# cbacary/MoDeGPT

Measured on AMD Instinct MI355X. Metric: transformer layers compressed/sec (covariance+decomp+rebuild), Llama-3-8B @30%, higher is better.
Workload: dtype f64 from int8 MFMA digit planes, exact route: nine plane pairs + fp64 remainder sums, nothing truncated (error <= 5e-15 per call: fp64 rounding)

## Files before the change

### modegpt_amd/csrc/common.hpp

```cpp
#pragma once
#include <hip/hip_runtime.h>
#include <hip/hip_bf16.h>
#include <hip/hip_fp16.h>
#include <stdint.h>
#include <stdio.h>
#include <string.h>

#include "../../include/modegpt_hip.h"

namespace mdg {

typedef double d4 __attribute__((ext_vector_type(4)));
typedef double d2 __attribute__((ext_vector_type(2)));
typedef unsigned short bf16_t;
typedef unsigned short f16_t;

#ifdef MDG_EXPERIMENT
#define MDG_KNOB(name) (getenv(name) != nullptr)
#else
#define MDG_KNOB(name) false
#endif

void set_error(const char* fmt, ...);
enum { STATUS_NOT_PD = 1, STATUS_NO_CONVERGE = 2 };
int finish_flag(int* dflag, hipStream_t st, int kind, const char* what);

int release_i8_schedules();
int cov_accum_gated(const void* x, int dtype, int64_t n_tokens, int64_t n_feat, int64_t batch, int64_t ld, int relu, double* sigma,
                    int64_t ld_sigma, int64_t sigma_bs, void* ws, size_t ws_bytes, const int* gate, int gate_mask, int gate_want,
                    void* stream);
#define MDG_CHECK_ARG(cond, ...)            \
  do {                                      \
    if (!(cond)) {                          \
      mdg::set_error(__VA_ARGS__);          \
      return MDG_ERR_BAD_ARG;               \
    }                                       \
  } while (0)
#define MDG_HIP(call)                                                        \
  do {                                                                       \
    hipError_t e_ = (call);                                                  \
    if (e_ != hipSuccess) {                                                  \
      mdg::set_error("%s failed: %s (%s:%d)", #call, hipGetErrorString(e_),  \
                     __FILE__, __LINE__);                                    \
      return MDG_ERR_HIP;                                                    \
    }                                                                        \
  } while (0)
#define MDG_LAUNCH_CHECK() MDG_HIP(hipGetLastError())
#define MDG_CLEAR() (void)hipGetLastError()
#define MDG_TRY(call)              \
  do {                             \
    int s_ = (call);               \
    if (s_ != MDG_OK) return s_;   \
  } while (0)

__device__ __forceinline__ double bf16_to_f64(bf16_t b) {
  return (double)__uint_as_float(((unsigned)b) << 16);
}
__device__ __forceinline__ double f16_to_f64(f16_t h) {
  __half_raw r;
  r.x = h;
  return (double)__half2float(__half(r));
}
__device__ __forceinline__ bf16_t f64_to_bf16(double v) {
  float f = (float)v;
  unsigned u = __float_as_uint(f);
  if ((u & 0x7fffffffu) > 0x7f800000u) return (bf16_t)0x7fc0;
  u += 0x7fffu + ((u >> 16) & 1u);
  return (bf16_t)(u >> 16);
}

template <int DT> struct ElemOf;
template <> struct ElemOf<MDG_BF16> { typedef bf16_t type; };
template <> struct ElemOf<MDG_F16> { typedef f16_t type; };
template <> struct ElemOf<MDG_F32> { typedef float type; };
template <> struct ElemOf<MDG_F64> { typedef double type; };

template <int DT> __device__ __forceinline__ double load_f64(const void* p, int64_t i);
template <> __device__ __forceinline__ double load_f64<MDG_BF16>(const void* p, int64_t i) {
  return bf16_to_f64(((const bf16_t*)p)[i]);
}
template <> __device__ __forceinline__ double load_f64<MDG_F16>(const void* p, int64_t i) {
  return f16_to_f64(((const f16_t*)p)[i]);
}
template <> __device__ __forceinline__ double load_f64<MDG_F32>(const void* p, int64_t i) {
  return (double)((const float*)p)[i];
}
template <> __device__ __forceinline__ double load_f64<MDG_F64>(const void* p, int64_t i) {
  return ((const double*)p)[i];
}

static inline size_t dtype_size(int dt) {
  switch (dt) {
    case MDG_BF16: case MDG_F16: return 2;
    case MDG_F32: return 4;
    case MDG_F64: return 8;
  }
  return 0;
}

static inline int64_t ceil_div(int64_t a, int64_t b) { return (a + b - 1) / b; }
static inline size_t align_up(size_t a, size_t b) { return (a + b - 1) / b * b; }

constexpr int TILE = 128;
constexpr int WTILE = 64;
constexpr int BK = 16;
constexpr int PITCH = TILE + 2;
constexpr int PANEL = BK * PITCH;

struct Acc {
  d4 v[4][4];
};

__device__ __forceinline__ void acc_zero(Acc& a) {
#pragma unroll
  for (int i = 0; i < 4; i++)
#pragma unroll
    for (int j = 0; j < 4; j++) a.v[i][j] = (d4){0., 0., 0., 0.};
}

template <int K4_LO, int K4_HI>
__device__ __forceinline__ void mma_steps(const double* __restrict__ As, const double* __restrict__ Bs, int wr,
                                          int wc, int lane, Acc& acc) {
  const int m = lane & 15, kq = lane >> 4;
#pragma unroll
  for (int k4 = K4_LO; k4 < K4_HI; k4++) {
    const double* ap = As + (k4 * 4 + kq) * PITCH + wr * WTILE + 4 * m;
    const double* bp = Bs + (k4 * 4 + kq) * PITCH + wc * WTILE + 4 * m;
    d2 a01 = *(const d2*)ap, a23 = *(const d2*)(ap + 2);
    d2 b01 = *(const d2*)bp, b23 = *(const d2*)(bp + 2);
    double a[4] = {a01.x, a01.y, a23.x, a23.y};
    double b[4] = {b01.x, b01.y, b23.x, b23.y};
#pragma unroll
    for (int sa = 0; sa < 4; sa++)
#pragma unroll
      for (int sb = 0; sb < 4; sb++)
        acc.v[sa][sb] = __builtin_amdgcn_mfma_f64_16x16x4f64(a[sa], b[sb], acc.v[sa][sb], 0, 0, 0);
  }
}

__device__ __forceinline__ void mma_stage(const double* __restrict__ As, const double* __restrict__ Bs, int wr,
                                          int wc, int lane, Acc& acc) {
  mma_steps<0, BK / 4>(As, Bs, wr, wc, lane, acc);
}

__device__ __forceinline__ int acc_row(int wr, int lane, int sa, int reg) {
  return wr * WTILE + 4 * ((lane >> 4) + 4 * reg) + sa;
}
__device__ __forceinline__ int acc_col(int wc, int lane, int sb) { return wc * WTILE + 4 * (lane & 15) + sb; }

__device__ __forceinline__ void tri_decode(int t, int& bi, int& bj) {
  int i = (int)((sqrt(8.0 * (double)t + 1.0) - 1.0) * 0.5);
  while ((i + 1) * (i + 2) / 2 <= t) i++;
  while (i * (i + 1) / 2 > t) i--;
  bi = i;
  bj = t - i * (i + 1) / 2;
}

}
```

### modegpt_amd/csrc/cov.hip

```cpp
#include <stdlib.h>

#include <type_traits>

#include "common.hpp"

namespace mdg {

struct CovArgs {
  const void* x;
  int64_t ld, n_tokens;
  int n_feat, batch, tiles, ntri;
  double* sigma;
  int64_t ld_sigma, sigma_bs;
  int ksplit;
  int64_t tokens_per_split;
  double* partial;
  int vec_ok;
  const int* gate;
  int gate_mask, gate_want;
};

template <int DT> struct Stage {
  typedef typename ElemOf<DT>::type T;
  static constexpr int VEC = 16 / (int)sizeof(T);
  static constexpr int CPR = TILE / VEC;
  static constexpr int CPT = BK * CPR / 256;
  union Chunk {
    uint4 q;
    T e[VEC];
  };
  static constexpr int RG = VEC >= 8 ? 4 : (VEC == 4 ? 2 : 1);
  static constexpr int CG = 8 / RG;
  __device__ static __forceinline__ void chunk_rc(int c, int& row, int& col) {
    const int g = c >> 3, i = c & 7;
    row = (g % (BK / RG)) * RG + (i % RG);
    col = ((g / (BK / RG)) * CG + i / RG) * VEC;
  }
};

template <int DT, bool FAST, bool INB = false>
__device__ __forceinline__ void load_panel(const CovArgs& a, int64_t tok0, int64_t tok_end, int64_t col0,
                                           int col_lim, int tid, typename Stage<DT>::Chunk* regs) {
  typedef Stage<DT> S;
  typedef typename S::T T;
  const T* x = (const T*)a.x;
#pragma unroll
  for (int p = 0; p < S::CPT; p++) {
    int row, col;
    S::chunk_rc(tid + 256 * p, row, col);
    int64_t tok = tok0 + row;
    typename S::Chunk ch;
    ch.q = make_uint4(0, 0, 0, 0);
    if (FAST && INB) {
      ch.q = *(const uint4*)(x + tok * a.ld + col0 + col);
    } else if (FAST) {
      if (tok < tok_end) ch.q = *(const uint4*)(x + tok * a.ld + col0 + col);
    } else if (tok < tok_end) {
      const T* src = x + tok * a.ld + col0 + col;
      if (a.vec_ok && col + S::VEC <= col_lim) {
        ch.q = *(const uint4*)src;
      } else {
#pragma unroll
        for (int e = 0; e < S::VEC; e++)
          if (col + e < col_lim) ch.e[e] = src[e];
      }
    }
    regs[p] = ch;
  }
}

template <int DT, bool RELU>
__device__ __forceinline__ void store_panel(double* panel, int tid, const typename Stage<DT>::Chunk* regs) {
  typedef Stage<DT> S;
#pragma unroll
  for (int p = 0; p < S::CPT; p++) {
    int row, col;
    S::chunk_rc(tid + 256 * p, row, col);
    double* dst = panel + row * PITCH + col;
#pragma unroll
    for (int e = 0; e < S::VEC; e += 2) {
      double v0 = load_f64<DT>(regs[p].e, e), v1 = load_f64<DT>(regs[p].e, e + 1);
      if (RELU) {
        v0 = v0 > 0. ? v0 : 0.;
        v1 = v1 > 0. ? v1 : 0.;
      }
      *(d2*)(dst + e) = (d2){v0, v1};
    }
  }
}

template <int DT, bool RELU>
__device__ __forceinline__ void store_piece(double* panel, int tid, const typename Stage<DT>::Chunk* regs, int piece) {
  typedef Stage<DT> S;
  constexpr int PAIRS = S::CPT * S::VEC / 2;
  constexpr int PER = PAIRS / 4;
#pragma unroll
  for (int u = 0; u < PER; u++) {
    const int w = piece * PER + u;
    const int p = w / (S::VEC / 2), e = (w % (S::VEC / 2)) * 2;
    int row, col;
    S::chunk_rc(tid + 256 * p, row, col);
    double v0 = load_f64<DT>(regs[p].e, e), v1 = load_f64<DT>(regs[p].e, e + 1);
    if (RELU) {
      v0 = v0 > 0. ? v0 : 0.;
      v1 = v1 > 0. ? v1 : 0.;
    }
    *(d2*)(panel + row * PITCH + col + e) = (d2){v0, v1};
  }
}

template <int DT, bool RELU, bool DIAG>
__device__ __forceinline__ void mma_half_with_staging(const double* __restrict__ As, const double* __restrict__ Bs,
                                                      int wr, int wc, int lane, Acc& acc, bool stage_next,
                                                      double* nextA, double* nextB, int tid,
                                                      const typename Stage<DT>::Chunk* ra,
                                                      const typename Stage<DT>::Chunk* rb) {
  const int m = lane & 15, kq = lane >> 4;
  double a[2][4], b[2][4];
#pragma unroll
  for (int h = 0; h < 2; h++) {
    const int k4 = BK / 8 + h;
    const double* ap = As + (k4 * 4 + kq) * PITCH + wr * WTILE + 4 * m;
    const double* bp = Bs + (k4 * 4 + kq) * PITCH + wc * WTILE + 4 * m;
    d2 a01 = *(const d2*)ap, a23 = *(const d2*)(ap + 2);
    d2 b01 = *(const d2*)bp, b23 = *(const d2*)(bp + 2);
    a[h][0] = a01.x; a[h][1] = a01.y; a[h][2] = a23.x; a[h][3] = a23.y;
    b[h][0] = b01.x; b[h][1] = b01.y; b[h][2] = b23.x; b[h][3] = b23.y;
  }
#pragma unroll
  for (int h = 0; h < 2; h++)
#pragma unroll
    for (int sa = 0; sa < 4; sa++) {
#pragma unroll
      for (int sb = 0; sb < 4; sb++)
        acc.v[sa][sb] = __builtin_amdgcn_mfma_f64_16x16x4f64(a[h][sa], b[h][sb], acc.v[sa][sb], 0, 0, 0);
      if (stage_next) {
        const int piece = h * 4 + sa;
        if (piece < 4) store_piece<DT, RELU>(nextA, tid, ra, piece);
        else if (!DIAG) store_piece<DT, RELU>(nextB, tid, rb, piece - 4);
      }
      __builtin_amdgcn_sched_barrier(0);
    }
}

template <int DT, bool RELU, bool FAST, bool DIAG>
__device__ __forceinline__ void cov_tile(const CovArgs& a, double* lds, int b, int bi, int bj, int split, int slot) {
  typedef Stage<DT> S;
  const int tid = threadIdx.x, lane = tid & 63, wave = tid >> 6;
  const int wr = wave >> 1, wc = wave & 1;
  const int64_t tok_begin = (int64_t)split * a.tokens_per_split;
  int64_t tok_end = tok_begin + a.tokens_per_split;
  if (tok_end > a.n_tokens) tok_end = a.n_tokens;
  const int64_t colA = (int64_t)b * a.n_feat + (int64_t)bi * TILE;
  const int64_t colB = (int64_t)b * a.n_feat + (int64_t)bj * TILE;
  const int limA = min(TILE, a.n_feat - bi * TILE), limB = min(TILE, a.n_feat - bj * TILE);

  Acc acc;
  acc_zero(acc);
  typename S::Chunk ra1[S::CPT], rb1[S::CPT], ra2[S::CPT], rb2[S::CPT];
  const int64_t n_stage = tok_end > tok_begin ? (tok_end - tok_begin + BK - 1) / BK : 0;

  if (n_stage > 0) {
    load_panel<DT, FAST>(a, tok_begin, tok_end, colA, limA, tid, ra1);
    if (!DIAG) load_panel<DT, FAST>(a, tok_begin, tok_end, colB, limB, tid, rb1);
    store_panel<DT, RELU>(lds, tid, ra1);
    if (!DIAG) store_panel<DT, RELU>(lds + 2 * PANEL, tid, rb1);
    if (n_stage > 1) {
      load_panel<DT, FAST>(a, tok_begin + BK, tok_end, colA, limA, tid, ra1);
      if (!DIAG) load_panel<DT, FAST>(a, tok_begin + BK, tok_end, colB, limB, tid, rb1);
    }
  }
  __syncthreads();
  auto stage = [&](int64_t s, auto cur_c, auto steady_c, typename S::Chunk* st_a, typename S::Chunk* st_b,
                   typename S::Chunk* ld_a, typename S::Chunk* ld_b) {
    constexpr int CUR = decltype(cur_c)::value;
    constexpr bool STEADY = decltype(steady_c)::value;
    if (STEADY || s + 2 < n_stage) {
      const int64_t tk = tok_begin + (s + 2) * BK;
      load_panel<DT, FAST, STEADY>(a, tk, tok_end, colA, limA, tid, ld_a);
      if (!DIAG) load_panel<DT, FAST, STEADY>(a, tk, tok_end, colB, limB, tid, ld_b);
    }
    const double* As = lds + CUR * PANEL;
    const double* Bs = DIAG ? As : lds + (2 + CUR) * PANEL;
    mma_steps<0, BK / 8>(As, Bs, wr, wc, lane, acc);
    mma_half_with_staging<DT, RELU, DIAG>(As, Bs, wr, wc, lane, acc, STEADY || s + 1 < n_stage, lds + (CUR ^ 1) * PANEL,
                                          lds + (2 + (CUR ^ 1)) * PANEL, tid, st_a, st_b);
    __syncthreads();
  };
  using I0 = std::integral_constant<int, 0>;
  using I1 = std::integral_constant<int, 1>;
  int64_t s = 0;
  const int64_t n_full = (tok_end - tok_begin) / BK;
  for (; s + 3 < n_full; s += 2) {
    stage(s, I0{}, std::true_type{}, ra1, rb1, ra2, rb2);
    stage(s + 1, I1{}, std::true_type{}, ra2, rb2, ra1, rb1);
  }
  for (; s + 1 < n_stage; s += 2) {
    stage(s, I0{}, std::false_type{}, ra1, rb1, ra2, rb2);
    stage(s + 1, I1{}, std::false_type{}, ra2, rb2, ra1, rb1);
  }
  if (s < n_stage) stage(s, I0{}, std::false_type{}, ra1, rb1, ra2, rb2);

  if (a.ksplit == 1) {
    double* sg = a.sigma + (int64_t)b * a.sigma_bs;
#pragma unroll
    for (int sa = 0; sa < 4; sa++)
#pragma unroll
      for (int reg = 0; reg < 4; reg++) {
        int r = acc_row(wr, lane, sa, reg);
        int64_t gr = (int64_t)bi * TILE + r;
        if (gr >= a.n_feat) continue;
        int c0 = acc_col(wc, lane, 0);
        int64_t gc0 = (int64_t)bj * TILE + c0;
        double* row = sg + gr * a.ld_sigma + gc0;
#pragma unroll
        for (int sb = 0; sb < 4; sb++)
          if (gc0 + sb < a.n_feat) row[sb] += acc.v[sa][sb][reg];
      }
  } else {
    double* pt = a.partial + ((int64_t)split * (a.batch * a.ntri) + slot) * (TILE * TILE);
#pragma unroll
    for (int sa = 0; sa < 4; sa++)
#pragma unroll
      for (int reg = 0; reg < 4; reg++) {
        int r = acc_row(wr, lane, sa, reg);
        int c0 = acc_col(wc, lane, 0);
        d4 v = {acc.v[sa][0][reg], acc.v[sa][1][reg], acc.v[sa][2][reg], acc.v[sa][3][reg]};
        *(d4*)(pt + r * TILE + c0) = v;
      }
  }
}

template <int DT, bool RELU, bool FAST>
__global__ __launch_bounds__(256, 2) void cov_accum_kernel(CovArgs a) {
  __shared__ double lds[4 * PANEL];
  if (a.gate && (*a.gate & a.gate_mask) != a.gate_want) return;
  const int b = blockIdx.x / a.ntri, t = blockIdx.x % a.ntri;
  int bi, bj;
  tri_decode(t, bi, bj);
  if (bi == bj) cov_tile<DT, RELU, FAST, true>(a, lds, b, bi, bj, blockIdx.y, blockIdx.x);
  else cov_tile<DT, RELU, FAST, false>(a, lds, b, bi, bj, blockIdx.y, blockIdx.x);
}

constexpr int MULTI_MAX = 4;
struct CovMulti {
  int n;
  int unit_start[MULTI_MAX + 1];
  CovArgs p[MULTI_MAX];
};

template <int DT>
__global__ __launch_bounds__(256, 2) void cov_accum_multi_kernel(CovMulti m) {
  __shared__ double lds[4 * PANEL];
  int u = blockIdx.x, pi = 0;
  while (pi + 1 < m.n && u >= m.unit_start[pi + 1]) pi++;
  u -= m.unit_start[pi];
  const CovArgs& a = m.p[pi];
  const int tiles = a.batch * a.ntri;
  const int split = u / tiles, slot = u % tiles;
  const int b = slot / a.ntri, t = slot % a.ntri;
  int bi, bj;
  tri_decode(t, bi, bj);
  if (bi == bj) cov_tile<DT, false, true, true>(a, lds, b, bi, bj, split, slot);
  else cov_tile<DT, false, true, false>(a, lds, b, bi, bj, split, slot);
}

__global__ __launch_bounds__(256) void cov_reduce_kernel(CovArgs a) {
  if (a.gate && (*a.gate & a.gate_mask) != a.gate_want) return;
  const int b = blockIdx.x / a.ntri, t = blockIdx.x % a.ntri;
  int bi, bj;
  tri_decode(t, bi, bj);
  double* sg = a.sigma + (int64_t)b * a.sigma_bs;
  const int64_t tile_stride = (int64_t)gridDim.x * (TILE * TILE);
  const double* pt = a.partial + (int64_t)blockIdx.x * (TILE * TILE);
  const int e = blockIdx.y * 256 + threadIdx.x;
  const int r = e / TILE, c = e % TILE;
  const int64_t gr = (int64_t)bi * TILE + r, gc = (int64_t)bj * TILE + c;
  if (gr >= a.n_feat || gc >= a.n_feat) return;
  double s = 0.;
  for (int k = 0; k < a.ksplit; k++) s += pt[k * tile_stride + e];
  sg[gr * a.ld_sigma + gc] += s;
}

__global__ __launch_bounds__(256) void cov_finalize_kernel(double* sigma, int n, int64_t ld, int64_t bs, int tiles,
                                                           int ntri, double scale) {
  __shared__ double tl[32][33];
  const int b = blockIdx.x / ntri, t = blockIdx.x % ntri;
  int ti, tj;
  tri_decode(t, ti, tj);
  double* sg = sigma + (int64_t)b * bs;
  const int tx = threadIdx.x & 31, ty = threadIdx.x >> 5;
  for (int r = ty; r < 32; r += 8) {
    int gr = ti * 32 + r, gc = tj * 32 + tx;
    tl[r][tx] = (gr < n && gc < n) ? sg[(int64_t)gr * ld + gc] * scale : 0.;
  }
  __syncthreads();
  for (int r = ty; r < 32; r += 8) {
    int gr = ti * 32 + r, gc = tj * 32 + tx;
    if (gr < n && gc < n) {
      double v = (ti == tj && tx > r) ? tl[tx][r] : tl[r][tx];
      sg[(int64_t)gr * ld + gc] = v;
    }
    if (ti != tj) {
      int ur = tj * 32 + r, uc = ti * 32 + tx;
      if (ur < n && uc < n) sg[(int64_t)ur * ld + uc] = tl[tx][r];
    }
  }
}

template <int DT>
__global__ __launch_bounds__(256) void bi_partial_kernel(const void* xin, const void* xout, int64_t n_tokens,
                                                         int64_t d, int64_t ld, double* partial) {
  __shared__ double red[4];
  const int lane = threadIdx.x & 63, wave = threadIdx.x >> 6;
  double local = 0.;
  for (int64_t tok = (int64_t)blockIdx.x * 4 + wave; tok < n_tokens; tok += (int64_t)gridDim.x * 4) {
    double dot = 0., na = 0., nb = 0.;
    for (int64_t j = lane; j < d; j += 64) {
      double u = load_f64<DT>(xin, tok * ld + j), v = load_f64<DT>(xout, tok * ld + j);
      dot += u * v;
      na += u * u;
      nb += v * v;
    }
    for (int o = 32; o > 0; o >>= 1) {
      dot += __shfl_xor(dot, o);
      na += __shfl_xor(na, o);
      nb += __shfl_xor(nb, o);
    }
    const double eps = 1e-8;
    double den = fmax(sqrt(na), eps) * fmax(sqrt(nb), eps);
    local += 1.0 - dot / den;
  }
  if (lane == 0) red[wave] = local;
  __syncthreads();
  if (threadIdx.x == 0) partial[blockIdx.x] = red[0] + red[1] + red[2] + red[3];
}

__global__ void bi_final_kernel(const double* partial, int n, double* out) {
  if (threadIdx.x == 0 && blockIdx.x == 0) {
    double s = 0.;
    for (int i = 0; i < n; i++) s += partial[i];
    *out += s;
  }
}

static int cov_ksplit(int64_t n_tokens, int64_t n_feat, int64_t batch, int64_t* tokens_per_split) {
  const int64_t T = ceil_div(n_feat, TILE);
  const int64_t blocks = batch * T * (T + 1) / 2;
  const double slots = 512.0;
  const double us_per_token = 2.0 * TILE * TILE / (78.6e12 / slots) * 1e6;
  const double us_per_tile_rt = 2.0 * TILE * TILE * 8 / 4.0e12 * 1e6;
  int64_t max_split = n_tokens / (8 * BK);
  if (max_split < 1) max_split = 1;
  if (max_split > 256) max_split = 256;
  int64_t best = 1;
  double best_cost = 0.;
#ifdef MDG_EXPERIMENT
  if (const char* ev = getenv("MDG_COV_KSPLIT")) {
    const int64_t f = atoll(ev);
    if (f >= 1 && f <= max_split) {
      const int64_t tps = (int64_t)align_up((size_t)ceil_div(n_tokens, f), BK);
      *tokens_per_split = tps;
      return (int)ceil_div(n_tokens, tps);
    }
  }
#endif
  for (int64_t ks = 1; ks <= max_split; ks++) {
    const int64_t tps = (int64_t)align_up((size_t)ceil_div(n_tokens, ks), BK);
    const int64_t real = ceil_div(n_tokens, tps);
    if (real != ks) continue;
    double rounds = (double)ceil_div(blocks * ks, (int64_t)slots);
    double cost = rounds * (double)tps * us_per_token + (ks > 1 ? (double)(blocks * ks) * us_per_tile_rt + 3.0 : 0.);
    if (ks == 1 || cost < best_cost * (best == 1 ? 0.95 : 0.98)) {
      best = ks;
      best_cost = cost;
    }
  }
  int64_t tps = (int64_t)align_up((size_t)ceil_div(n_tokens > 0 ? n_tokens : 1, best), BK);
  *tokens_per_split = tps;
  return (int)ceil_div(n_tokens > 0 ? n_tokens : 1, tps);
}

template <int DT>
static void launch_cov(const CovArgs& a, int relu, bool fast, hipStream_t st) {
  dim3 grid(a.batch * a.ntri, a.ksplit);
  if (fast) {
    if (relu) hipLaunchKernelGGL((cov_accum_kernel<DT, true, true>), grid, dim3(256), 0, st, a);
    else hipLaunchKernelGGL((cov_accum_kernel<DT, false, true>), grid, dim3(256), 0, st, a);
  } else {
    if (relu) hipLaunchKernelGGL((cov_accum_kernel<DT, true, false>), grid, dim3(256), 0, st, a);
    else hipLaunchKernelGGL((cov_accum_kernel<DT, false, false>), grid, dim3(256), 0, st, a);
  }
}

}

using namespace mdg;

extern "C" size_t mdg_cov_accum_ws_bytes(int64_t n_tokens, int64_t n_feat, int64_t batch) {
  if (n_tokens <= 0 || n_feat <= 0 || batch <= 0) return 0;
  int64_t tps;
  int ks = cov_ksplit(n_tokens, n_feat, batch, &tps);
  if (ks == 1) return 0;
  int64_t T = ceil_div(n_feat, TILE);
  return (size_t)ks * batch * (T * (T + 1) / 2) * TILE * TILE * sizeof(double);
}

extern "C" int mdg_cov_accum(const void* x, int dtype, int64_t n_tokens, int64_t n_feat, int64_t batch,
                             int64_t ld, int relu, double* sigma, int64_t ld_sigma, int64_t sigma_bs, void* ws,
                             size_t ws_bytes, void* stream) {
  return mdg::cov_accum_gated(x, dtype, n_tokens, n_feat, batch, ld, relu, sigma, ld_sigma, sigma_bs, ws, ws_bytes, nullptr, 0, 0,
                              stream);
}

int mdg::cov_accum_gated(const void* x, int dtype, int64_t n_tokens, int64_t n_feat, int64_t batch, int64_t ld, int relu,
                         double* sigma, int64_t ld_sigma, int64_t sigma_bs, void* ws, size_t ws_bytes, const int* gate,
                         int gate_mask, int gate_want, void* stream) {
  MDG_CLEAR();
  MDG_CHECK_ARG(n_tokens >= 0 && n_feat > 0 && batch > 0, "mdg_cov_accum: bad sizes (tokens=%lld feat=%lld batch=%lld)",
                (long long)n_tokens, (long long)n_feat, (long long)batch);
  MDG_CHECK_ARG(dtype >= MDG_BF16 && dtype <= MDG_F64, "mdg_cov_accum: unknown dtype %d", dtype);
  MDG_CHECK_ARG(ld >= n_feat * batch, "mdg_cov_accum: ld %lld < batch*n_feat %lld", (long long)ld,
                (long long)(n_feat * batch));
  MDG_CHECK_ARG(ld_sigma >= n_feat, "mdg_cov_accum: ld_sigma %lld < n_feat", (long long)ld_sigma);
  MDG_CHECK_ARG(batch == 1 || sigma_bs >= n_feat * ld_sigma - (ld_sigma - n_feat),
                "mdg_cov_accum: sigma batch stride too small");
  MDG_CHECK_ARG(n_feat < (1 << 30) && batch * n_feat < (1ll << 31), "mdg_cov_accum: n_feat too large");
  if (n_tokens == 0) return MDG_OK;
  MDG_CHECK_ARG(x && sigma, "mdg_cov_accum: null pointer");
  hipStream_t st = (hipStream_t)stream;
  CovArgs a;
  a.x = x;
  a.ld = ld;
  a.n_tokens = n_tokens;
  a.n_feat = (int)n_feat;
  a.batch = (int)batch;
  a.tiles = (int)ceil_div(n_feat, TILE);
  a.ntri = a.tiles * (a.tiles + 1) / 2;
  a.sigma = sigma;
  a.ld_sigma = ld_sigma;
  a.sigma_bs = sigma_bs;
  a.ksplit = cov_ksplit(n_tokens, n_feat, batch, &a.tokens_per_split);
  a.partial = (double*)ws;
  a.gate = gate;
  a.gate_mask = gate_mask;
  a.gate_want = gate_want;
  size_t esz = dtype_size(dtype);
  a.vec_ok = ((uintptr_t)x % 16 == 0) && ((ld * esz) % 16 == 0) && ((n_feat * esz) % 16 == 0 || batch == 1);
  if (a.ksplit > 1) {
    size_t need = mdg_cov_accum_ws_bytes(n_tokens, n_feat, batch);
    MDG_CHECK_ARG(ws && ws_bytes >= need, "mdg_cov_accum: workspace %zu < required %zu", ws_bytes, need);
  }
  MDG_CHECK_ARG((int64_t)a.batch * a.ntri < (1ll << 31) && a.ksplit < 65536, "mdg_cov_accum: grid too large");
  const bool fast = a.vec_ok && (n_feat % TILE == 0);
  switch (dtype) {
    case MDG_BF16: launch_cov<MDG_BF16>(a, relu, fast, st); break;
    case MDG_F16: launch_cov<MDG_F16>(a, relu, fast, st); break;
    case MDG_F32: launch_cov<MDG_F32>(a, relu, fast, st); break;
    default: launch_cov<MDG_F64>(a, relu, fast, st); break;
  }
  MDG_LAUNCH_CHECK();
  if (a.ksplit > 1) {
    hipLaunchKernelGGL(cov_reduce_kernel, dim3(a.batch * a.ntri, TILE * TILE / 256), dim3(256), 0, st, a);
    MDG_LAUNCH_CHECK();
  }
  return MDG_OK;
}

static int multi_ksplit(int64_t n_tokens, int64_t* tokens_per_split) {
  int64_t ks = n_tokens / 4096;
  if (ks < 1) ks = 1;
  if (ks > 64) ks = 64;
  int64_t tps = (int64_t)align_up((size_t)ceil_div(n_tokens, ks), BK);
  *tokens_per_split = tps;
  return (int)ceil_div(n_tokens, tps);
}

static int multi_plan(int n, const mdg_cov_problem* pr, int dtype, CovMulti* m, size_t* ws_need) {
  MDG_CHECK_ARG(n >= 1 && n <= MULTI_MAX && pr, "mdg_cov_accum_multi: 1..%d problems", MULTI_MAX);
  MDG_CHECK_ARG(dtype >= MDG_BF16 && dtype <= MDG_F64, "mdg_cov_accum_multi: unknown dtype %d", dtype);
  const size_t esz = dtype_size(dtype);
  size_t off = 0;
  int64_t units = 0;
  m->n = n;
  for (int i = 0; i < n; i++) {
    const mdg_cov_problem& q = pr[i];
    MDG_CHECK_ARG(q.n_tokens > 0 && q.n_feat > 0 && q.batch > 0 && q.x && q.sigma, "mdg_cov_accum_multi: problem %d empty", i);
    MDG_CHECK_ARG(q.n_feat % TILE == 0 && q.ld >= q.n_feat * q.batch && q.ld_sigma >= q.n_feat,
                  "mdg_cov_accum_multi: problem %d needs n_feat %% 128 == 0 (got %lld) and consistent strides", i,
                  (long long)q.n_feat);
    MDG_CHECK_ARG((uintptr_t)q.x % 16 == 0 && (q.ld * esz) % 16 == 0,
                  "mdg_cov_accum_multi: problem %d is not 16-byte aligned (use mdg_cov_accum)", i);
    CovArgs& a = m->p[i];
    a.x = q.x; a.ld = q.ld; a.n_tokens = q.n_tokens; a.n_feat = (int)q.n_feat; a.batch = (int)q.batch;
    a.tiles = (int)(q.n_feat / TILE); a.ntri = a.tiles * (a.tiles + 1) / 2;
    a.sigma = q.sigma; a.ld_sigma = q.ld_sigma; a.sigma_bs = q.sigma_batch_stride; a.vec_ok = 1;
    a.gate = nullptr; a.gate_mask = a.gate_want = 0;
    const int64_t tiles = (int64_t)a.batch * a.ntri;
    if (i == 0 && tiles >= 768) { a.ksplit = 1; a.tokens_per_split = (int64_t)align_up((size_t)q.n_tokens, BK); }
    else a.ksplit = multi_ksplit(q.n_tokens, &a.tokens_per_split);
    a.partial = nullptr;
    m->unit_start[i] = (int)units;
    units += tiles * a.ksplit;
    MDG_CHECK_ARG(units < (1ll << 30), "mdg_cov_accum_multi: grid too large");
    if (a.ksplit > 1) {
      a.partial = (double*)off;
      off += (size_t)a.ksplit * tiles * TILE * TILE * sizeof(double);
    }
  }
  m->unit_start[n] = (int)units;
  *ws_need = off;
  return MDG_OK;
}

extern "C" size_t mdg_cov_accum_multi_ws_bytes(int n, const mdg_cov_problem* problems, int dtype) {
  CovMulti m;
  size_t need = 0;
  if (multi_plan(n, problems, dtype, &m, &need) != MDG_OK) return 0;
  return need;
}

extern "C" int mdg_cov_accum_multi(int n, const mdg_cov_problem* problems, int dtype, void* ws, size_t ws_bytes,
                                   void* stream) {
  MDG_CLEAR();
  CovMulti m;
  size_t need = 0;
  MDG_TRY(multi_plan(n, problems, dtype, &m, &need));
  MDG_CHECK_ARG(need == 0 || (ws && ws_bytes >= need), "mdg_cov_accum_multi: workspace %zu < required %zu", ws_bytes, need);
  for (int i = 0; i < n; i++)
    if (m.p[i].ksplit > 1) m.p[i].partial = (double*)((char*)ws + (size_t)m.p[i].partial);
  hipStream_t st = (hipStream_t)stream;
  dim3 grid((unsigned)m.unit_start[n]);
  switch (dtype) {
    case MDG_BF16: hipLaunchKernelGGL(cov_accum_multi_kernel<MDG_BF16>, grid, dim3(256), 0, st, m); break;
    case MDG_F16: hipLaunchKernelGGL(cov_accum_multi_kernel<MDG_F16>, grid, dim3(256), 0, st, m); break;
    case MDG_F32: hipLaunchKernelGGL(cov_accum_multi_kernel<MDG_F32>, grid, dim3(256), 0, st, m); break;
    default: hipLaunchKernelGGL(cov_accum_multi_kernel<MDG_F64>, grid, dim3(256), 0, st, m); break;
  }
  MDG_LAUNCH_CHECK();
  for (int i = 0; i < n; i++)
    if (m.p[i].ksplit > 1) {
      hipLaunchKernelGGL(cov_reduce_kernel, dim3(m.p[i].batch * m.p[i].ntri, TILE * TILE / 256), dim3(256), 0, st, m.p[i]);
      MDG_LAUNCH_CHECK();
    }
  return MDG_OK;
}

extern "C" int mdg_cov_finalize(double* sigma, int64_t n, int64_t batch, int64_t ld_sigma, int64_t sigma_bs,
                                double scale, void* stream) {
  MDG_CLEAR();
  MDG_CHECK_ARG(sigma && n > 0 && batch > 0 && ld_sigma >= n, "mdg_cov_finalize: bad arguments");
  int tiles = (int)ceil_div(n, 32);
  int64_t ntri = (int64_t)tiles * (tiles + 1) / 2;
  MDG_CHECK_ARG(batch * ntri < (1ll << 31), "mdg_cov_finalize: grid too large");
  hipLaunchKernelGGL(cov_finalize_kernel, dim3((unsigned)(batch * ntri)), dim3(256), 0, (hipStream_t)stream, sigma,
                     (int)n, ld_sigma, sigma_bs, tiles, (int)ntri, scale);
  MDG_LAUNCH_CHECK();
  return MDG_OK;
}

static const int BI_MAX_BLOCKS = 2048;
extern "C" size_t mdg_bi_ws_bytes(int64_t n_tokens) { return (size_t)BI_MAX_BLOCKS * sizeof(double); }

extern "C" int mdg_bi_accum(const void* x_in, const void* x_out, int dtype, int64_t n_tokens, int64_t d, int64_t ld,
                            double* out, void* ws, size_t ws_bytes, void* stream) {
  MDG_CLEAR();
  MDG_CHECK_ARG(x_in && x_out && out && n_tokens >= 0 && d > 0 && ld >= d, "mdg_bi_accum: bad arguments");
  MDG_CHECK_ARG(ws && ws_bytes >= mdg_bi_ws_bytes(n_tokens), "mdg_bi_accum: workspace too small");
  if (n_tokens == 0) return MDG_OK;
  int blocks = (int)(ceil_div(n_tokens, 4) < BI_MAX_BLOCKS ? ceil_div(n_tokens, 4) : BI_MAX_BLOCKS);
  hipStream_t st = (hipStream_t)stream;
  double* partial = (double*)ws;
  switch (dtype) {
    case MDG_BF16: hipLaunchKernelGGL(bi_partial_kernel<MDG_BF16>, dim3(blocks), dim3(256), 0, st, x_in, x_out, n_tokens, d, ld, partial); break;
    case MDG_F16: hipLaunchKernelGGL(bi_partial_kernel<MDG_F16>, dim3(blocks), dim3(256), 0, st, x_in, x_out, n_tokens, d, ld, partial); break;
    case MDG_F32: hipLaunchKernelGGL(bi_partial_kernel<MDG_F32>, dim3(blocks), dim3(256), 0, st, x_in, x_out, n_tokens, d, ld, partial); break;
    case MDG_F64: hipLaunchKernelGGL(bi_partial_kernel<MDG_F64>, dim3(blocks), dim3(256), 0, st, x_in, x_out, n_tokens, d, ld, partial); break;
    default: MDG_CHECK_ARG(false, "mdg_bi_accum: unknown dtype %d", dtype);
  }
  MDG_LAUNCH_CHECK();
  hipLaunchKernelGGL(bi_final_kernel, dim3(1), dim3(64), 0, st, partial, blocks, out);
  MDG_LAUNCH_CHECK();
  return MDG_OK;
}
```

### modegpt_amd/csrc/cov_i8.hip

```cpp
#include <algorithm>

#include "cov_i8.hpp"

namespace mdg {
namespace {

size_t layout(int count, const mdg_cov_problem* pr, void* ws, I8Call* out, size_t* fallback_off) {
  size_t off = SHARED_BYTES + PARTIAL_BYTES, fb = 0;
  char* const base = (char*)ws;
  if (out) {
    out->count = count;
    out->n_tokens = pr[0].n_tokens;
    out->nk = (int)ceil_div(pr[0].n_tokens, KS);
    out->shared = (SharedBlock*)base;
    out->partial = (double*)(base + SHARED_BYTES);
  }
  for (int i = 0; i < count; i++) {
    const int64_t cols = pr[i].n_feat * pr[i].batch, T = pr[i].n_tokens;
    const LoWsBytes lo = lo_ws_bytes(T, cols);
    I8Stat s;
    s.x = (const bf16_t*)pr[i].x; s.ld = pr[i].ld;
    s.sigma = pr[i].sigma; s.ld_sigma = pr[i].ld_sigma;
    s.n = (int)cols; s.block = pr[i].batch > 1 ? TI : 0;
    s.route_flag = out ? out->shared->route_flag + i : nullptr;
    auto take = [&](size_t bytes) { char* p = base ? base + off : nullptr; off += bytes; return p; };
    s.planes = (signed char*)take(align_up((size_t)NP * (size_t)cols * (size_t)ceil_div(T, KS) * KS, 256));
    s.emax = (int*)take(align_up(ints_bytes(cols), 256));
    s.vals = (double*)take(align_up(route_vals_bytes(cols), 256));
    s.route = (RouteOut*)take(align_up(sizeof(RouteOut), 256));
    s.colpart = (double*)take(align_up(column_partials_bytes(cols), 256));
    s.zmask = (unsigned char*)take(align_up((size_t)ceil_div(T, KS) * (size_t)(cols / 32), 256));
    s.lo_entries = (LoEntry*)take(lo.entries);
    s.lo_counts = (int*)take(align_up(lo.counts, 256));
    s.lo_xd = (bf16_t*)take(align_up(lo.xd, 256));
    s.lo_rentries = (LoEntry*)take(lo.rentries);
    s.lo_rtotals = (int*)take(align_up(lo.rtotals, 256));
    if (out) out->stat[i] = s;
    fb = std::max(fb, mdg_cov_accum_ws_bytes(T, pr[i].n_feat, pr[i].batch));
  }
  if (fallback_off) *fallback_off = off;
  return off + fb + 256;
}

bool problems_ok(int count, const mdg_cov_problem* pr) {
  if (count < 1 || count > MAX_PROBLEMS || !pr) return false;
  for (int i = 0; i < count; i++) {
    if (pr[i].n_tokens != pr[0].n_tokens || pr[i].n_tokens < 0 || pr[i].n_tokens >= (1ll << 28) || pr[i].n_feat <= 0 || pr[i].batch < 1) return false;
    if (pr[i].batch == 1 ? pr[i].n_feat % TI != 0 : pr[i].n_feat != TI) return false;
    if (pr[i].n_feat * pr[i].batch >= (1 << 21)) return false;
    if (pr[i].ld < pr[i].n_feat * pr[i].batch || pr[i].ld_sigma < pr[i].n_feat) return false;
    if (pr[i].batch > 1 && (pr[i].ld_sigma != TI || pr[i].sigma_batch_stride != (int64_t)TI * TI)) return false;
  }
  return true;
}

}
}

using namespace mdg;

extern "C" size_t mdg_cov_accum_i8_multi_ws_bytes(int count, const mdg_cov_problem* problems) {
  if (!problems_ok(count, problems) || problems[0].n_tokens == 0) return 0;
  return layout(count, problems, nullptr, nullptr, nullptr);
}

extern "C" int mdg_cov_accum_i8_multi(int count, const mdg_cov_problem* problems, void* ws, size_t ws_bytes, double tolerance, int flags,
                                      int* used_i8, int* route_counts, void* ev_start, void* ev_stop, void* stream) {
  MDG_CLEAR();
  if (used_i8) *used_i8 = 0;
  MDG_CHECK_ARG(tolerance >= 1.0 && tolerance <= 1e6, "mdg_cov_accum_i8_multi: tolerance factor %g outside [1, 1e6] (1 = guaranteed <= 1.1e-11)",
                tolerance);
  MDG_CHECK_ARG((flags & ~(MDG_I8_NO_EXACT | MDG_I8_EXACT_ALWAYS | MDG_I8_F16 | MDG_I8_RELU)) == 0 &&
                    (flags & (MDG_I8_NO_EXACT | MDG_I8_EXACT_ALWAYS)) != (MDG_I8_NO_EXACT | MDG_I8_EXACT_ALWAYS),
                "mdg_cov_accum_i8_multi: bad flags 0x%x", flags);
  bool offer_exact = !(flags & MDG_I8_NO_EXACT);
  const bool exact_always = (flags & MDG_I8_EXACT_ALWAYS) != 0;
  for (int i = 0; i < count; i++)
    if ((uint64_t)problems[i].n_tokens * (uint64_t)problems[i].ld * 2ull >= (1ull << 32)) offer_exact = false;
  MDG_CHECK_ARG(problems_ok(count, problems),
                "mdg_cov_accum_i8_multi: 1..%d statistics of the same token count; full ones need n_feat %% 128 == 0, per-head ones "
                "head_dim 128 with contiguous [heads][128][128] sigma; leading dimensions at least the widths (use mdg_cov_accum)",
                MAX_PROBLEMS);
  if (problems[0].n_tokens == 0) return MDG_OK;
  for (int i = 0; i < count; i++) MDG_CHECK_ARG(problems[i].x && problems[i].sigma, "mdg_cov_accum_i8_multi: null pointer");
  I8Call c;
  size_t fb_off = 0;
  const size_t need = layout(count, problems, ws, &c, &fb_off);
  MDG_CHECK_ARG(ws && ws_bytes >= need, "mdg_cov_accum_i8_multi: workspace %zu < required %zu", ws_bytes, need);
  c.route_counts = route_counts;
  c.st = (hipStream_t)stream;
  c.f16 = (flags & MDG_I8_F16) != 0;
  c.relu = (flags & MDG_I8_RELU) != 0;
  MDG_HIP(hipMemsetAsync(c.shared, 0, SHARED_BYTES, c.st));
  for (int i = 0; i < count; i++) {
    MDG_TRY(enqueue_split(c, i));
    MDG_TRY(enqueue_route(c, i, tolerance));
  }
  if (offer_exact) MDG_TRY(enqueue_lo_lists(c, exact_always));
  MDG_TRY(enqueue_products(c, offer_exact, ev_start, ev_stop));
  if (offer_exact) MDG_TRY(enqueue_lo_products(c, exact_always));
  for (int i = 0; i < count; i++) MDG_TRY(enqueue_columns(c, i));
  for (int i = 0; i < count; i++) {
    const mdg_cov_problem& q = problems[i];
    MDG_TRY(cov_accum_gated(q.x, c.f16 ? MDG_F16 : MDG_BF16, c.n_tokens, q.n_feat, q.batch, q.ld, c.relu ? 1 : 0, q.sigma, q.ld_sigma, q.sigma_batch_stride, (char*)ws + fb_off,
                            ws_bytes - fb_off, c.stat[i].route_flag, 2, 2, stream));
  }
  MDG_TRY(report_product_diagnostics(c));
  if (used_i8) {
    int pf[MAX_PROBLEMS] = {};
    MDG_HIP(hipMemcpyAsync(pf, c.shared->route_flag, sizeof(pf), hipMemcpyDeviceToHost, c.st));
    MDG_HIP(hipStreamSynchronize(c.st));
    int live = 0, six = 0;
    for (int i = 0; i < count; i++)
      if (!(pf[i] & 2)) {
        live++;
        six |= pf[i] & 1;
      }
    *used_i8 = live ? (six ? 6 : 5) : 0;
  }
  return MDG_OK;
}

static mdg_cov_problem single_problem(const void* x, int64_t n_tokens, int64_t n_feat, int64_t ld, double* sigma, int64_t ld_sigma) {
  mdg_cov_problem q;
  q.x = x; q.n_tokens = n_tokens; q.n_feat = n_feat; q.batch = 1; q.ld = ld;
  q.sigma = sigma; q.ld_sigma = ld_sigma; q.sigma_batch_stride = 0;
  return q;
}

extern "C" size_t mdg_cov_accum_i8_ws_bytes(int64_t n_tokens, int64_t n_feat) {
  if (n_tokens <= 0 || n_feat <= 0) return 0;
  const mdg_cov_problem q = single_problem(nullptr, n_tokens, n_feat, n_feat, nullptr, n_feat);
  return mdg_cov_accum_i8_multi_ws_bytes(1, &q);
}

extern "C" int mdg_cov_accum_i8(const void* x, int64_t n_tokens, int64_t n_feat, int64_t ld, double* sigma, int64_t ld_sigma,
                                void* ws, size_t ws_bytes, double tolerance, int flags, int* used_i8, int* route_counts, void* ev_start,
                                void* ev_stop, void* stream) {
  MDG_CLEAR();
  if (used_i8) *used_i8 = 0;
  MDG_CHECK_ARG(n_tokens >= 0 && n_feat > 0, "mdg_cov_accum_i8: bad sizes (tokens=%lld feat=%lld)", (long long)n_tokens,
                (long long)n_feat);
  MDG_CHECK_ARG(n_feat % TI == 0, "mdg_cov_accum_i8: n_feat=%lld must be a multiple of %d (use mdg_cov_accum)",
                (long long)n_feat, TI);
  const mdg_cov_problem q = single_problem(x, n_tokens, n_feat, ld, sigma, ld_sigma);
  return mdg_cov_accum_i8_multi(1, &q, ws, ws_bytes, tolerance, flags, used_i8, route_counts, ev_start, ev_stop, stream);
}

extern "C" int mdg_cov_accum_i8_route(int count, const mdg_cov_problem* problems, int stat, const void* ws, int* planes, int* n_columns,
                                      int* columns, double* bound, int* exact, void* stream) {
  MDG_CLEAR();
  MDG_CHECK_ARG(problems_ok(count, problems) && stat >= 0 && stat < count && ws, "mdg_cov_accum_i8_route: bad arguments");
  I8Call c;
  layout(count, problems, const_cast<void*>(ws), &c, nullptr);
  RouteOut r;
  SharedBlock shared;
  hipStream_t st = (hipStream_t)stream;
  MDG_HIP(hipMemcpyAsync(&r, c.stat[stat].route, sizeof(r), hipMemcpyDeviceToHost, st));
  MDG_HIP(hipMemcpyAsync(&shared, c.shared, sizeof(shared), hipMemcpyDeviceToHost, st));
  MDG_HIP(hipStreamSynchronize(st));
  const bool was_exact = r.planes != 0 && shared.exact_ran == 1 && shared.exact_overflow == 0;
  if (exact) *exact = was_exact ? shared.exact_mode : 0;
  if (planes) *planes = r.planes;
  if (n_columns) *n_columns = r.n_out;
  if (columns)
    for (int i = 0; i < MDG_I8_MAX_COLUMNS; i++) columns[i] = i < r.n_out ? r.out[i] : -1;
  if (bound) {
    bound[0] = was_exact ? r.rho + MDG_I8_EXACT_ROUNDING : r.sq;
    bound[1] = was_exact ? 0.0 : r.x;
  }
  return MDG_OK;
}

extern "C" int mdg_cov_accum_i8_stats(const void* ws, int64_t n_tokens, int64_t n_feat, unsigned long long* executed_mfma,
                                      void* stream) {
  MDG_CLEAR();
  (void)n_tokens;
  (void)n_feat;
  MDG_CHECK_ARG(ws && executed_mfma, "mdg_cov_accum_i8_stats: bad arguments");
  const SharedBlock* shared = (const SharedBlock*)ws;
  hipStream_t st = (hipStream_t)stream;
  MDG_HIP(hipMemcpyAsync(executed_mfma, &shared->mfma_count, sizeof(unsigned long long), hipMemcpyDeviceToHost, st));
  MDG_HIP(hipStreamSynchronize(st));
  return MDG_OK;
}
```

### modegpt_amd/csrc/cov_i8.hpp

```cpp
#pragma once
#include <cstddef>

#include "common.hpp"

namespace mdg {

typedef int i32x4 __attribute__((ext_vector_type(4)));

constexpr int NP = 6;
constexpr int TI = 128;
constexpr int KS = 32;
constexpr int FLUSH_STEPS = 2047;
constexpr int FLUSH_STEPS_F16 = 2047;
static_assert(FLUSH_STEPS <= FLUSH_STEPS_F16, "the product kernels' fold interval must hold for fp16 elements too");
constexpr int TOP_SHIFT = 8 * NP - 10;
constexpr int TOP_SHIFT_F16 = 8 * NP - 13;

struct Bf16Elem {
  static constexpr int TOP = TOP_SHIFT, SIG_BITS = 8;
  static __device__ __forceinline__ void parts(unsigned b, int& sig, int& ee) {
    const int e = (b >> 7) & 0xFF, m = b & 0x7F;
    sig = e ? (128 | m) : m;
    ee = e ? e : 1;
    if (b & 0x8000) sig = -sig;
  }
  static __device__ __forceinline__ int ee_if_nonzero(unsigned b) {
    const int e = (b >> 7) & 0xFF;
    return (b & 0x7FFF) ? (e ? e : 1) : 0;
  }
  static __device__ __forceinline__ bool is_nan(unsigned b) { return (b & 0x7FFFu) > 0x7F80u; }
  static __device__ __forceinline__ double to_f64(unsigned b) { return (double)__uint_as_float(b << 16); }
  static __device__ __forceinline__ double lo_f64(unsigned w) { return (double)__uint_as_float(w << 16); }
  static __device__ __forceinline__ double hi_f64(unsigned w) { return (double)__uint_as_float(w & 0xFFFF0000u); }
  static __device__ __forceinline__ unsigned from_f64(double v) { return __float_as_uint((float)v) >> 16; }
  static __device__ __forceinline__ unsigned deep_limit(int E) { return (unsigned)max(E - 14, 1) << 7; }
};
struct F16Elem {
  static constexpr int TOP = TOP_SHIFT_F16, SIG_BITS = 11;
  static __device__ __forceinline__ void parts(unsigned b, int& sig, int& ee) {
    const int e = (b >> 10) & 0x1F, m = b & 0x3FF;
    sig = e ? (1024 | m) : m;
    ee = e == 31 ? 255 : (e ? e : 1) + 112;
    if (b & 0x8000) sig = -sig;
  }
  static __device__ __forceinline__ int ee_if_nonzero(unsigned b) {
    const int e = (b >> 10) & 0x1F;
    return (b & 0x7FFF) ? (e == 31 ? 255 : (e ? e : 1) + 112) : 0;
  }
  static __device__ __forceinline__ bool is_nan(unsigned b) { return (b & 0x7FFFu) > 0x7C00u; }
  static __device__ __forceinline__ double to_f64(unsigned b) { return f16_to_f64((f16_t)b); }
  static __device__ __forceinline__ double lo_f64(unsigned w) { return f16_to_f64((f16_t)(w & 0xFFFFu)); }
  static __device__ __forceinline__ double hi_f64(unsigned w) { return f16_to_f64((f16_t)(w >> 16)); }
  static __device__ __forceinline__ unsigned from_f64(double v) { return __half_as_ushort(__float2half((float)v)); }
  static __device__ __forceinline__ unsigned deep_limit(int E) { return (unsigned)max(E - 123, 1) << 10; }
};
template <class EL, bool RELU>
__device__ __forceinline__ unsigned relu_bits(unsigned b) {
  return (RELU && (b & 0x8000u) && !EL::is_nan(b)) ? 0u : b;
}
template <class EL, bool RELU>
__device__ __forceinline__ unsigned relu_pair(unsigned w) {
  if (!RELU) return w;
  return relu_bits<EL, true>(w & 0xFFFFu) | (relu_bits<EL, true>(w >> 16) << 16);
}
#define MDG_I8_DISPATCH(c, KERNEL, ...)                                                   \
  do {                                                                                    \
    if ((c).f16) {                                                                        \
      if ((c).relu) hipLaunchKernelGGL((KERNEL<F16Elem, true>), __VA_ARGS__);             \
      else hipLaunchKernelGGL((KERNEL<F16Elem, false>), __VA_ARGS__);                     \
    } else {                                                                              \
      if ((c).relu) hipLaunchKernelGGL((KERNEL<Bf16Elem, true>), __VA_ARGS__);            \
      else hipLaunchKernelGGL((KERNEL<Bf16Elem, false>), __VA_ARGS__);                    \
    }                                                                                     \
  } while (0)

constexpr int NSTAT = 8;
constexpr int STAT_D0D1 = 6, STAT_COUNTS = 7;
constexpr int EMAX_COLUMN_OUT = 0x100;

constexpr int ALWAYS_WRITTEN_PLANES = 4;

constexpr int MAX_PROBLEMS = 4;
constexpr int ROUTE_JMAX = MDG_I8_MAX_COLUMNS;
constexpr int TAIL_MAX_PIECES = 1024;
constexpr size_t PARTIAL_BYTES = (size_t)TAIL_MAX_PIECES * TI * 128 * sizeof(double);

struct RouteOut {
  int planes;
  int n_out;
  int out[ROUTE_JMAX];
  double sq, x;
  double rho;
};
struct RouteScratch {
  int ticket, forced;
};

constexpr size_t SHARED_BYTES = 256;
struct SharedBlock {
  int reserved[2];
  unsigned long long mfma_count;
  int xcd_queue[8];
  int route_flag[MAX_PROBLEMS];
  int exact_overflow, exact_ran, exact_mode;
};
static_assert(offsetof(SharedBlock, mfma_count) == 8 && offsetof(SharedBlock, xcd_queue) == 16 && offsetof(SharedBlock, route_flag) == 48 &&
                  offsetof(SharedBlock, exact_overflow) == 64 && offsetof(SharedBlock, exact_ran) == 68 &&
                  offsetof(SharedBlock, exact_mode) == 72 && sizeof(SharedBlock) <= SHARED_BYTES,
              "the shared block's layout is fixed");

struct LoEntry;
struct I8Stat {
  const bf16_t* x;
  int64_t ld;
  double* sigma;
  int64_t ld_sigma;
  int n, block;
  int* route_flag;
  signed char* planes;
  int* emax;
  unsigned char* zmask;
  double* vals;
  RouteOut* route;
  double* colpart;
  LoEntry *lo_entries, *lo_rentries;
  int *lo_counts, *lo_rtotals;
  bf16_t* lo_xd;
  bool vec() const { return (uintptr_t)x % 16 == 0 && ld % 8 == 0; }
  unsigned long long* stats() const { return (unsigned long long*)(emax + (n + 1) / 2 * 2); }
};
struct I8Call {
  int count, nk;
  int64_t n_tokens;
  I8Stat stat[MAX_PROBLEMS];
  bool f16, relu;
  SharedBlock* shared;
  double* partial;
  int* route_counts;
  hipStream_t st;
};

inline size_t ints_bytes(int64_t n) { return (size_t)((n + 1) / 2 * 2) * sizeof(int) + (size_t)(NSTAT * n) * sizeof(unsigned long long) + sizeof(RouteScratch); }

#pragma GCC visibility push(hidden)
int enqueue_split(const I8Call& c, int i);
size_t route_vals_bytes(int64_t n);
size_t column_partials_bytes(int64_t n);
int enqueue_route(const I8Call& c, int i, double tolerance);
int enqueue_columns(const I8Call& c, int i);
struct LoWsBytes { size_t entries, counts, xd, rentries, rtotals; };
LoWsBytes lo_ws_bytes(int64_t n_tokens, int64_t n);
int enqueue_lo_lists(const I8Call& c, bool always);
int enqueue_lo_products(const I8Call& c, bool always);
int enqueue_products(const I8Call& c, bool offer_exact, void* ev_start, void* ev_stop);
int report_product_diagnostics(const I8Call& c);
#pragma GCC visibility pop

}
```

### modegpt_amd/csrc/cov_i8_route.hip

```cpp
#include <algorithm>

#include "cov_i8.hpp"

namespace mdg {
namespace {

constexpr double TAU_SQ = 1e-12, TAU_X_MIN = 1e-12, TAU_X_MAX = 1e-11, TAU_X_TOKENS = 1024.0;
__host__ __device__ inline double tau_x_of(int64_t tokens) {
  return fmin(TAU_X_MAX, fmax(TAU_X_MIN, TAU_X_MIN * ((double)tokens / TAU_X_TOKENS)));
}
constexpr int NVAL = 7;
constexpr int ROUTE_THREADS = 512;

__device__ __forceinline__ void route_terms(const double (&A)[NVAL], int P, double& sq, double& x) {
  sq = 2.0 * A[6] + A[6] * A[6];
  x = 0.0;
#pragma unroll
  for (int s = 0; s < NP; s++)
#pragma unroll
    for (int t = 0; t < NP; t++)
      if (s + t >= P) {
        if (s == t) sq += A[s] * A[t];
        else x += A[s] * A[t];
      }
}
__device__ __forceinline__ double route_violation(const double (&A)[NVAL], int P, double tau_x) {
  double sq, x;
  route_terms(A, P, sq, x);
  return fmax(sq / TAU_SQ, x / tau_x);
}

struct Top2 { double m1; int a1; double m2; };
__device__ __forceinline__ void top2_merge(Top2& a, const Top2& b) {
  if (b.m1 > a.m1 || (b.m1 == a.m1 && b.a1 < a.a1)) {
    a.m2 = fmax(a.m1, b.m2);
    a.m1 = b.m1;
    a.a1 = b.a1;
  } else {
    a.m2 = fmax(a.m2, b.m1);
  }
}

struct RoutePartial {
  Top2 top[NVAL];
  unsigned long long cls[NVAL][64];
  unsigned min_nnz;
};

__global__ __launch_bounds__(ROUTE_THREADS) void i8_route_kernel(const unsigned long long* __restrict__ stats, int* emax, int n, int64_t n_tokens,
                                                                 double* __restrict__ vals, RoutePartial* partial, RouteScratch* scratch,
                                                                 int* flag, RouteOut* out, int* route_counts, double tolerance) {
  __shared__ unsigned long long group_max[NVAL][64];
  __shared__ Top2 wave_top[ROUTE_THREADS / 64][NVAL];
  __shared__ Top2 top[NVAL];
  __shared__ double floor_of[NVAL];
  __shared__ int decision;
  __shared__ int forced_total, my_ticket;
  __shared__ unsigned min_nnz;
  __shared__ double tau_x_shared;
  const int tid = threadIdx.x, lane = tid & 63, wave = tid >> 6;
  for (int i = tid; i < NVAL * 64; i += ROUTE_THREADS) (&group_max[0][0])[i] = 0ull;
  if (tid == 0) min_nnz = 0xffffffffu;
  __syncthreads();
  auto reduce_top = [&](Top2 (&t)[NVAL]) {
#pragma unroll
    for (int i = 0; i < NVAL; i++) {
#pragma unroll
      for (int off = 32; off >= 1; off >>= 1) {
        Top2 o;
        o.m1 = __shfl_xor(t[i].m1, off);
        o.a1 = __shfl_xor(t[i].a1, off);
        o.m2 = __shfl_xor(t[i].m2, off);
        top2_merge(t[i], o);
      }
      if (lane == 0) wave_top[wave][i] = t[i];
    }
    __syncthreads();
    if (tid < NVAL) {
      Top2 r = wave_top[0][tid];
      for (int w = 1; w < ROUTE_THREADS / 64; w++) top2_merge(r, wave_top[w][tid]);
      top[tid] = r;
    }
    __syncthreads();
  };
  Top2 t[NVAL];
#pragma unroll
  for (int i = 0; i < NVAL; i++) t[i] = Top2{-1.0, 0x7fffffff, -1.0};
  {
    const int j = blockIdx.x * ROUTE_THREADS + tid;
    bool nonfinite = false;
    if (j < n) {
      double q[NSTAT];
#pragma unroll
      for (int i = 0; i < NSTAT - 1; i++) q[i] = i == STAT_D0D1 ? (double)(long long)stats[(int64_t)i * n + j] : (double)stats[(int64_t)i * n + j];
      const unsigned long long counts = stats[(int64_t)STAT_COUNTS * n + j];
      const int ex = emax[j];
      const double nnz = (double)(unsigned)counts, rounded = (double)(unsigned)(counts >> 32);
      const double hi2 = 65536.0 * q[0] + 512.0 * q[STAT_D0D1] + q[1];
      const double norm = (sqrt(fmax(hi2, 0.0)) - 0.5 * sqrt(nnz)) * 4294967296.0;
      const double inv = nnz > 0 ? (norm > 0 ? 1.0 / norm : 1e300) : 0.0;
      double a[NVAL];
#pragma unroll
      for (int s2 = 0; s2 < NP; s2++) a[s2] = q[s2] > 0 ? sqrt(q[s2]) * ldexp(1.0, 8 * (NP - 1 - s2)) * inv : 0.0;
      a[6] = rounded > 0 ? 0.5 * sqrt(rounded) * inv : 0.0;
      nonfinite = (ex & 255) == 255;
      if ((unsigned)counts) atomicMin(&min_nnz, (unsigned)counts);
#pragma unroll
      for (int i = 0; i < NVAL; i++) {
        vals[(int64_t)i * n + j] = a[i];
        if (!nonfinite) t[i] = Top2{a[i], j, -1.0};
      }
      if (nonfinite) emax[j] = ex | EMAX_COLUMN_OUT;
    }
#pragma unroll
    for (int i = 0; i < NVAL; i++)
      if (t[i].m1 > 0.0) atomicMax(&group_max[i][lane], (unsigned long long)__double_as_longlong(t[i].m1));
    const unsigned long long nf = __ballot(nonfinite);
    if (lane == 0 && nf) atomicAdd(&scratch->forced, __popcll(nf));
  }
  reduce_top(t);
  RoutePartial& mine = partial[blockIdx.x];
  if (tid < NVAL) mine.top[tid] = top[tid];
  if (tid == 0) mine.min_nnz = min_nnz;
  for (int i = tid; i < NVAL * 64; i += ROUTE_THREADS) (&mine.cls[0][0])[i] = (&group_max[0][0])[i];
  __threadfence();
  __syncthreads();
  if (tid == 0) my_ticket = atomicAdd(&scratch->ticket, 1);
  __syncthreads();
  if (my_ticket != (int)gridDim.x - 1) return;
  __threadfence();
  const unsigned nwg = gridDim.x;
  if (tid < NVAL) {
    Top2 r = partial[0].top[tid];
    unsigned w = 1;
    for (; w + 4 <= nwg; w += 4) {
      const Top2 b0 = partial[w].top[tid], b1 = partial[w + 1].top[tid], b2 = partial[w + 2].top[tid], b3 = partial[w + 3].top[tid];
      top2_merge(r, b0); top2_merge(r, b1); top2_merge(r, b2); top2_merge(r, b3);
    }
    for (; w < nwg; w++) top2_merge(r, partial[w].top[tid]);
    r.m1 = fmax(r.m1, 0.0);
    r.m2 = fmax(r.m2, 0.0);
    top[tid] = r;
  }
  for (int i = tid; i < NVAL * 64; i += ROUTE_THREADS) {
    unsigned long long m = 0ull;
    unsigned w = 0;
    for (; w + 4 <= nwg; w += 4) {
      const unsigned long long v0 = (&partial[w].cls[0][0])[i], v1 = (&partial[w + 1].cls[0][0])[i], v2 = (&partial[w + 2].cls[0][0])[i],
                               v3 = (&partial[w + 3].cls[0][0])[i];
      m = max(max(m, v0), max(max(v1, v2), v3));
    }
    for (; w < nwg; w++) m = max(m, (&partial[w].cls[0][0])[i]);
    (&group_max[0][0])[i] = m;
  }
  if (tid == 0) {
    forced_total = scratch->forced;
    unsigned m = 0xffffffffu;
    unsigned w = 0;
    for (; w + 4 <= nwg; w += 4) {
      const unsigned v0 = partial[w].min_nnz, v1 = partial[w + 1].min_nnz, v2 = partial[w + 2].min_nnz, v3 = partial[w + 3].min_nnz;
      m = min(min(m, v0), min(min(v1, v2), v3));
    }
    for (; w < nwg; w++) m = min(m, partial[w].min_nnz);
    tau_x_shared = tau_x_of(min(n_tokens, (int64_t)m));
  }
  __syncthreads();
  const double tau_x = tau_x_shared;
  int n_out = 0;
  if (forced_total > ROUTE_JMAX) {
    if (tid == 0) {
      out->planes = 0; out->n_out = 0; out->sq = out->x = out->rho = 0.0;
      atomicOr(flag, 2);
    }
    for (int j = tid; j < n; j += ROUTE_THREADS) emax[j] &= 255;
    return;
  }
  if (forced_total) {
    if (tid == 0)
      for (int j = 0; j < n; j++)
        if (emax[j] & EMAX_COLUMN_OUT) out->out[n_out++] = j;
    __syncthreads();
  }
  const int n_forced = forced_total;
  if (wave == 0) {
    const int want = ROUTE_JMAX - n_forced;
#pragma unroll 1
    for (int i = 0; i < NVAL; i++) {
      const unsigned long long mine = group_max[i][lane];
      int rank = 0;
      for (int k = 0; k < 64; k++) {
        const unsigned long long o = group_max[i][k];
        rank += (o > mine || (o == mine && k < lane));
      }
      if (rank == want) floor_of[i] = __longlong_as_double((long long)mine);
    }
  }
  __syncthreads();
  double fl[NVAL];
#pragma unroll
  for (int i = 0; i < NVAL; i++) fl[i] = floor_of[i];
  bool top_valid = true;
  for (int P = 5; P <= 6; P++) {
    if (n > 64 && route_violation(fl, P, tau_x) > tolerance) continue;
    n_out = n_forced;
    for (;;) {
      if (!top_valid) {
        top_valid = true;
#pragma unroll
        for (int i = 0; i < NVAL; i++) t[i] = Top2{-1.0, 0x7fffffff, -1.0};
        constexpr int PASS1_COLS = 4;
        for (int j0 = tid; j0 < n; j0 += ROUTE_THREADS * PASS1_COLS) {
          double v[PASS1_COLS][NVAL];
          int ex[PASS1_COLS];
#pragma unroll
          for (int c = 0; c < PASS1_COLS; c++) {
            const int j = j0 + c * ROUTE_THREADS;
            ex[c] = j < n ? emax[j] : EMAX_COLUMN_OUT;
#pragma unroll
            for (int i = 0; i < NVAL; i++) v[c][i] = j < n ? vals[(int64_t)i * n + j] : 0.0;
          }
#pragma unroll
          for (int c = 0; c < PASS1_COLS; c++)
            if (!(ex[c] & EMAX_COLUMN_OUT)) {
#pragma unroll
              for (int i = 0; i < NVAL; i++) top2_merge(t[i], Top2{v[c][i], j0 + c * ROUTE_THREADS, -1.0});
            }
        }
        reduce_top(t);
      }
      if (tid == 0) {
        double A[NVAL];
#pragma unroll
        for (int i = 0; i < NVAL; i++) {
          top[i].m1 = fmax(top[i].m1, 0.0);
          top[i].m2 = fmax(top[i].m2, 0.0);
          A[i] = top[i].m1;
        }
        decision = -1;
        if (route_violation(A, P, tau_x) <= tolerance) {
          out->planes = P;
          out->n_out = n_out;
          route_terms(A, P, out->sq, out->x);
          out->rho = 2.0 * A[6] + A[6] * A[6];
          if (P == 6) atomicOr(flag, 1);
          if (route_counts && n_out) atomicAdd(route_counts + 3, n_out);
          decision = 0;
        } else if (n_out == ROUTE_JMAX) {
          decision = 1;
        } else {
          int best = -1;
          double best_v = 1e308;
          for (int qi = 0; qi < NVAL; qi++) {
            const int c = top[qi].a1;
            if (c == 0x7fffffff) continue;
            double A2[NVAL];
#pragma unroll
            for (int i = 0; i < NVAL; i++) A2[i] = top[i].a1 == c ? top[i].m2 : top[i].m1;
            const double v = route_violation(A2, P, tau_x);
            if (v < best_v) { best_v = v; best = c; }
          }
          if (best < 0) decision = 1;
          else {
            emax[best] |= EMAX_COLUMN_OUT;
            out->out[n_out] = best;
          }
        }
      }
      __syncthreads();
      const int dec = decision;
      __syncthreads();
      if (dec == 0) return;
      if (dec == 1) break;
      n_out++;
      top_valid = false;
    }
    if (n_out > n_forced) {
      for (int j = tid; j < n; j += ROUTE_THREADS)
        if ((emax[j] & EMAX_COLUMN_OUT) && (emax[j] & 255) != 255) emax[j] &= 255;
      top_valid = false;
      __syncthreads();
    }
  }
  if (tid == 0) {
    out->planes = 0; out->n_out = 0; out->sq = out->x = out->rho = 0.0;
    atomicOr(flag, 2);
  }
  for (int j = tid; j < n; j += ROUTE_THREADS) emax[j] &= 255;
}

__global__ __launch_bounds__(256) void i8_clear_columns_kernel(const RouteOut* route, const int* flag, const int* emax, signed char* planes,
                                                               unsigned char* zmask, int n, int nk) {
  if ((*flag & 2) || (int)blockIdx.x >= route->n_out) return;
  const int j = route->out[blockIdx.x];
  const int64_t groups = n / 32;
  const int G = j >> 5, lane = threadIdx.x & 63, row = lane & 31;
  const bool row_out = (emax[G * 32 + row] & EMAX_COLUMN_OUT) != 0;
  for (int kt = blockIdx.y * 4 + (threadIdx.x >> 6); kt < nk; kt += gridDim.y * 4) {
    const unsigned old_mask = zmask[(int64_t)kt * groups + G];
    unsigned new_mask = 0;
#pragma unroll
    for (int s = 0; s < NP; s++) {
      if (s >= ALWAYS_WRITTEN_PLANES && (old_mask >> s) == 0) continue;
      i32x4* p = (i32x4*)(planes + ((s * groups + G) * (int64_t)nk + kt) * 1024) + lane;
      i32x4 v = *p;
      if (row_out) {
        v = (i32x4)0;
        *p = v;
      }
      if (__ballot((v[0] | v[1] | v[2] | v[3]) != 0)) new_mask |= 1u << s;
    }
    if (lane == 0) zmask[(int64_t)kt * groups + G] = (unsigned char)new_mask;
  }
}

constexpr int COLK_GROUP = 8, COLK_CHUNKS = 64, COLK_WG_COLS = 512, COLK_STAGE = 64, COLK_BATCH = 8;
struct ColArgs {
  const bf16_t* x;
  int64_t ld, T;
  int n, vec;
  const RouteOut* route;
  const int* flag;
  double* part;
};

template <class EL, bool RELU>
__global__ __launch_bounds__(64) void i8_columns_kernel(ColArgs a) {
  const int pass = blockIdx.z;
  const int n_out = a.route->n_out;
  if ((*a.flag & 2) || pass * COLK_GROUP >= n_out) return;
  const int nj = min(COLK_GROUP, n_out - pass * COLK_GROUP);
  __shared__ __attribute__((aligned(16))) double xj[COLK_STAGE][COLK_GROUP];
  const int lane = threadIdx.x;
  const int my_k = lane % COLK_GROUP;
  const int my_col = my_k < nj ? a.route->out[pass * COLK_GROUP + my_k] : -1;
  const int c0 = blockIdx.x * COLK_WG_COLS + lane * 8;
  const bool active = c0 < a.n;
  const int64_t chunk_len = (a.T + COLK_CHUNKS - 1) / COLK_CHUNKS;
  const int64_t t0 = blockIdx.y * chunk_len, t1 = min(a.T, t0 + chunk_len);
  const unsigned short* xs = (const unsigned short*)a.x;
  auto fetch_group = [&](int64_t t, unsigned short (&g)[COLK_STAGE / 8]) {
#pragma unroll
    for (int i = 0; i < COLK_STAGE / 8; i++) {
      const int64_t tok = t + lane / COLK_GROUP + 8 * i;
      g[i] = (my_col >= 0 && tok < t1) ? (unsigned short)relu_bits<EL, RELU>(xs[tok * a.ld + my_col]) : (unsigned short)0;
    }
  };
  double acc[COLK_GROUP][8] = {};
  unsigned short g[COLK_STAGE / 8];
  if (t0 < t1) fetch_group(t0, g);
  for (int64_t t = t0; t < t1; t += COLK_STAGE) {
    __syncthreads();
#pragma unroll
    for (int i = 0; i < COLK_STAGE / 8; i++) xj[lane / COLK_GROUP + 8 * i][my_k] = EL::to_f64(g[i]);
    __syncthreads();
    if (t + COLK_STAGE < t1) fetch_group(t + COLK_STAGE, g);
    if (!active) continue;
    const int steps = (int)min((int64_t)COLK_STAGE, t1 - t);
    for (int tb = 0; tb < steps; tb += COLK_BATCH) {
      unsigned w[COLK_BATCH][4];
#pragma unroll
      for (int i = 0; i < COLK_BATCH; i++) {
        const bool live = t + tb + i < t1;
        const int64_t tok = live ? t + tb + i : t1 - 1;
        if (a.vec) {
          const i32x4 v = *(const i32x4*)(xs + tok * a.ld + c0);
          w[i][0] = v[0]; w[i][1] = v[1]; w[i][2] = v[2]; w[i][3] = v[3];
        } else {
#pragma unroll
          for (int h = 0; h < 4; h++) w[i][h] = xs[tok * a.ld + c0 + 2 * h] | ((unsigned)xs[tok * a.ld + c0 + 2 * h + 1] << 16);
        }
        if (!live) w[i][0] = w[i][1] = w[i][2] = w[i][3] = 0u;
      }
#pragma unroll
      for (int i = 0; i < COLK_BATCH; i++) {
        double xc[8];
#pragma unroll
        for (int h = 0; h < 4; h++) {
          const unsigned wr = relu_pair<EL, RELU>(w[i][h]);
          xc[2 * h] = EL::to_f64(wr & 0xFFFFu);
          xc[2 * h + 1] = EL::to_f64(wr >> 16);
        }
#pragma unroll
        for (int k = 0; k < COLK_GROUP; k++) {
          const double xk = xj[tb + i][k];
#pragma unroll
          for (int c = 0; c < 8; c++) acc[k][c] += xk * xc[c];
        }
      }
    }
  }
  if (!active) return;
#pragma unroll
  for (int k = 0; k < COLK_GROUP; k++)
    if (k < nj) {
      double* o = a.part + ((int64_t)(pass * COLK_GROUP + k) * COLK_CHUNKS + blockIdx.y) * a.n + c0;
#pragma unroll
      for (int c = 0; c < 8; c++) o[c] = acc[k][c];
    }
}

__global__ __launch_bounds__(256) void i8_columns_reduce_kernel(ColArgs a, const int* emax, double* sigma, int64_t ld_sigma, int block) {
  const int k = blockIdx.y;
  if ((*a.flag & 2) || k >= a.route->n_out) return;
  const int c = blockIdx.x * 256 + threadIdx.x;
  if (c >= a.n) return;
  const int j = a.route->out[k];
  if (block && c / block != j / block) return;
  if ((emax[c] & EMAX_COLUMN_OUT) && c < j) return;
  double v = 0.0;
  for (int q = 0; q < COLK_CHUNKS; q++) v += a.part[((int64_t)k * COLK_CHUNKS + q) * a.n + c];
  const int row = max(c, j), col = min(c, j);
  sigma[(int64_t)row * ld_sigma + col - (block ? row / block * block : 0)] += v;
}

}

size_t route_vals_bytes(int64_t n) { return (size_t)(NVAL * n) * sizeof(double) + (size_t)ceil_div(n, (int64_t)ROUTE_THREADS) * sizeof(RoutePartial); }
size_t column_partials_bytes(int64_t n) { return (size_t)ROUTE_JMAX * COLK_CHUNKS * (size_t)n * sizeof(double); }

int enqueue_route(const I8Call& c, int i, double tolerance) {
  const I8Stat& s = c.stat[i];
  const int n = s.n;
  RoutePartial* partial = (RoutePartial*)(s.vals + (size_t)NVAL * n);
  RouteScratch* scratch = (RouteScratch*)(s.stats() + (size_t)NSTAT * n);
  hipLaunchKernelGGL(i8_route_kernel, dim3((unsigned)ceil_div(n, ROUTE_THREADS)), dim3(ROUTE_THREADS), 0, c.st, s.stats(), s.emax, n,
                     c.n_tokens, s.vals, partial, scratch, s.route_flag, s.route, c.route_counts, tolerance);
  hipLaunchKernelGGL(i8_clear_columns_kernel, dim3(ROUTE_JMAX, (unsigned)std::min(64, (c.nk + 3) / 4)), dim3(256), 0, c.st,
                     (const RouteOut*)s.route, (const int*)s.route_flag, (const int*)s.emax, s.planes, s.zmask, n, c.nk);
  MDG_LAUNCH_CHECK();
  return MDG_OK;
}

int enqueue_columns(const I8Call& c, int i) {
  const I8Stat& s = c.stat[i];
  ColArgs a;
  a.x = s.x; a.ld = s.ld; a.T = c.n_tokens; a.n = s.n;
  a.vec = s.vec();
  a.route = s.route;
  a.flag = s.route_flag;
  a.part = s.colpart;
  MDG_I8_DISPATCH(c, i8_columns_kernel, dim3((unsigned)ceil_div(s.n, COLK_WG_COLS), COLK_CHUNKS, ROUTE_JMAX / COLK_GROUP), dim3(64), 0, c.st, a);
  hipLaunchKernelGGL(i8_columns_reduce_kernel, dim3((unsigned)ceil_div(s.n, 256), ROUTE_JMAX), dim3(256), 0, c.st, a, (const int*)s.emax, s.sigma,
                     s.ld_sigma, s.block);
  MDG_LAUNCH_CHECK();
  return MDG_OK;
}

}
```

### modegpt_amd/csrc/cov_i8_split.hip

```cpp
#include <algorithm>

#include "cov_i8.hpp"

namespace mdg {
namespace {

template <class EL>
__device__ __forceinline__ long long fixed_point(int sig, int sh, bool& rounded) {
  rounded = sh > EL::TOP;
  if (!rounded) return (long long)sig << (EL::TOP - sh);
  const int dn = sh - EL::TOP;
  const int mag = dn > EL::SIG_BITS + 1 ? 0 : ((sig < 0 ? -sig : sig) + (1 << (dn - 1))) >> dn;
  return sig < 0 ? -mag : mag;
}

template <class EL, bool RELU>
__global__ __launch_bounds__(256) void i8_colmax_kernel(const bf16_t* x, int64_t ld, int64_t T, int n, int64_t rows_per_block,
                                                        int* emax) {
  const int j = blockIdx.x * 64 + (threadIdx.x & 63);
  const int64_t t0 = (int64_t)blockIdx.y * rows_per_block + (threadIdx.x >> 6);
  const int64_t t1 = min(T, (int64_t)(blockIdx.y + 1) * rows_per_block);
  int best = 1;
  if (j < n)
    for (int64_t t = t0; t < t1; t += 4) {
      int sig, ee;
      EL::parts(relu_bits<EL, RELU>(x[t * ld + j]), sig, ee);
      if (sig != 0) best = max(best, ee);
    }
  if (j < n) atomicMax(emax + j, best);
}

__device__ __forceinline__ unsigned write_piece_mask(const unsigned (&any)[NP], unsigned char* zmask, int64_t index) {
  unsigned byte = 0;
#pragma unroll
  for (int s = 0; s < NP; s++) {
    const unsigned long long b = __ballot(any[s] != 0);
    const unsigned half = (threadIdx.x & 32) ? (unsigned)(b >> 32) : (unsigned)b;
    byte |= (half != 0) << s;
  }
  if ((threadIdx.x & 31) == 0) zmask[index] = (unsigned char)byte;
  return byte;
}

constexpr int SPLIT_STEPS = 64;
template <class EL, bool RELU>
__global__ __launch_bounds__(256) void i8_split_kernel(const bf16_t* x, int64_t ld, int64_t T, int n, int nk, const int* emax,
                                                       signed char* planes, unsigned long long* stats, unsigned char* zmask) {
  __shared__ unsigned long long st_lds[NSTAT][32];
  const int r = threadIdx.x & 31;
  const int G = blockIdx.x;
  const int j = G * 32 + r;
  const int E = emax[j];
  const int64_t groups = n / 32;
  for (int i = threadIdx.x; i < NSTAT * 32; i += 256) (&st_lds[0][0])[i] = 0;
  __syncthreads();
  long long q[NSTAT] = {};
  for (int kq = 0; kq < SPLIT_STEPS; kq += 8) {
    const int kt = blockIdx.y * SPLIT_STEPS + kq + (threadIdx.x >> 5);
    if (kt >= nk) break;
    unsigned any[NP] = {};
#pragma unroll
    for (int h = 0; h < 2; h++) {
      unsigned dig[NP][4] = {};
#pragma unroll
      for (int qq = 0; qq < 16; qq++) {
        const int64_t t = (int64_t)kt * KS + h * 16 + qq;
        int sig = 0, ee = 1;
        if (t < T) EL::parts(relu_bits<EL, RELU>(x[t * ld + j]), sig, ee);
        bool rounded;
        long long N = fixed_point<EL>(sig, E - ee, rounded);
        q[STAT_COUNTS] += (long long)(sig != 0) + ((long long)(sig != 0 && rounded) << 32);
        int d[NP];
#pragma unroll
        for (int s = NP - 1; s >= 1; s--) {
          d[s] = (int)((N + 128) & 255) - 128;
          dig[s][qq >> 2] |= (unsigned)(d[s] & 255) << (8 * (qq & 3));
          N = (N - d[s]) >> 8;
        }
        d[0] = (int)N;
        dig[0][qq >> 2] |= (unsigned)(d[0] & 255) << (8 * (qq & 3));
#pragma unroll
        for (int s = 0; s < NP; s++) q[s] += d[s] * d[s];
        q[STAT_D0D1] += d[0] * d[1];
      }
#pragma unroll
      for (int s = 0; s < NP; s++) {
        signed char* piece = planes + ((s * groups + G) * (int64_t)nk + kt) * 1024;
        *(i32x4*)(piece + h * 512 + r * 16) = (i32x4){(int)dig[s][0], (int)dig[s][1], (int)dig[s][2], (int)dig[s][3]};
        any[s] |= dig[s][0] | dig[s][1] | dig[s][2] | dig[s][3];
      }
    }
    write_piece_mask(any, zmask, (int64_t)kt * groups + G);
  }
#pragma unroll
  for (int i = 0; i < NSTAT; i++)
    if (q[i]) atomicAdd(&st_lds[i][r], (unsigned long long)q[i]);
  __syncthreads();
  for (int i = threadIdx.x; i < NSTAT * 32; i += 256)
    if (st_lds[i >> 5][i & 31]) atomicAdd(stats + (int64_t)(i >> 5) * n + G * 32 + (i & 31), st_lds[i >> 5][i & 31]);
}

#ifndef MDG_COLMAX_WGS
#define MDG_COLMAX_WGS 4096
#endif
template <class EL, bool RELU>
__global__ __launch_bounds__(256) void i8_colmax_vec_kernel(const bf16_t* x, int64_t ld, int64_t T, int64_t rows_per_block, int* emax) {
  __shared__ int best_lds[128];
  const int cg = threadIdx.x & 15, tl = threadIdx.x >> 4;
  const int j0 = blockIdx.x * 128 + cg * 8;
  const int64_t t0 = (int64_t)blockIdx.y * rows_per_block + tl;
  const int64_t t1 = min(T, (int64_t)(blockIdx.y + 1) * rows_per_block);
  if (threadIdx.x < 128) best_lds[threadIdx.x] = 1;
  __syncthreads();
  int best[8] = {1, 1, 1, 1, 1, 1, 1, 1};
  for (int64_t t = t0; t < t1; t += 16) {
    const i32x4 v = *(const i32x4*)(x + t * ld + j0);
#pragma unroll
    for (int q = 0; q < 4; q++) {
      const unsigned w = relu_pair<EL, RELU>((unsigned)v[q]);
      best[2 * q] = max(best[2 * q], EL::ee_if_nonzero(w & 0xFFFF));
      best[2 * q + 1] = max(best[2 * q + 1], EL::ee_if_nonzero(w >> 16));
    }
  }
#pragma unroll
  for (int q = 0; q < 8; q++) atomicMax(&best_lds[cg * 8 + q], best[q]);
  __syncthreads();
  if (threadIdx.x < 128) atomicMax(emax + blockIdx.x * 128 + threadIdx.x, best_lds[threadIdx.x]);
}

constexpr int SPLIT_TILES = 8;
template <class EL, bool RELU>
__global__ __launch_bounds__(256) void i8_split_vec_kernel(const bf16_t* x, int64_t ld, int64_t T, int n, int nk, const int* emax,
                                                           signed char* planes, unsigned long long* stats, unsigned char* zmask) {
  __shared__ __attribute__((aligned(16))) bf16_t tile[64 * 128];
  __shared__ int st_lds[NSTAT + 1][128];
  const int f0 = blockIdx.x * 128;
  const int f = threadIdx.x & 127, ks = threadIdx.x >> 7;
  const int E = emax[f0 + f];
  const int64_t groups = n / 32;
  const int G = (f0 + f) >> 5, r = f & 31;
  for (int i = threadIdx.x; i < (NSTAT + 1) * 128; i += 256) (&st_lds[0][0])[i] = 0;
  int q[NSTAT + 1] = {};
  auto load_tile = [&](int tile_index, i32x4 (&v)[4]) {
    const int64_t tok0 = (int64_t)tile_index * 2 * KS;
#pragma unroll
    for (int c4 = 0; c4 < 4; c4++) {
      const int c = threadIdx.x + 256 * c4;
      const int64_t t = tok0 + (c >> 4);
      v[c4] = (i32x4)0;
      if (t < T) v[c4] = *(const i32x4*)(x + t * ld + f0 + (c & 15) * 8);
    }
  };
  const int tile0 = blockIdx.y * SPLIT_TILES, tiles = (nk + 1) / 2;
  for (int it = 0; it < SPLIT_TILES && tile0 + it < tiles; it++) {
    __syncthreads();
    {
      i32x4 v[4];
      load_tile(tile0 + it, v);
#pragma unroll
      for (int c4 = 0; c4 < 4; c4++) *(i32x4*)(tile + (threadIdx.x + 256 * c4) * 8) = v[c4];
    }
    __syncthreads();
    const int kt = (tile0 + it) * 2 + ks;
    if (kt >= nk) continue;
    unsigned any[NP] = {};
    unsigned deep_dig[2][NP - ALWAYS_WRITTEN_PLANES][4];
#pragma unroll
    for (int h = 0; h < 2; h++) {
      unsigned dig[NP][4];
#pragma unroll
      for (int q4 = 0; q4 < 4; q4++) {
        unsigned lo[4], hi[4];
#pragma unroll
        for (int e = 0; e < 4; e++) {
          int sig, ee;
          EL::parts(relu_bits<EL, RELU>(tile[(ks * 32 + h * 16 + q4 * 4 + e) * 128 + f]), sig, ee);
          q[NSTAT - 1] += (sig != 0);
          bool rounded;
          const long long N = fixed_point<EL>(sig, E - ee, rounded);
          if (rounded) q[NSTAT] += (sig != 0);
          const unsigned long long biased = (unsigned long long)N + 0x0000008080808080ull;
          lo[e] = (unsigned)biased;
          hi[e] = (unsigned)(biased >> 32);
        }
#pragma unroll
        for (int s2 = 0; s2 < NP; s2++) {
          constexpr unsigned ZERO_HI = 0x0c0c0000u;
          const int byte = NP - 1 - s2;
          const unsigned sel = ZERO_HI | (unsigned)(byte & 3) | ((4u + (unsigned)(byte & 3)) << 8);
          const unsigned t01 = __builtin_amdgcn_perm(byte < 4 ? lo[1] : hi[1], byte < 4 ? lo[0] : hi[0], sel);
          const unsigned t23 = __builtin_amdgcn_perm(byte < 4 ? lo[3] : hi[3], byte < 4 ? lo[2] : hi[2], sel);
          unsigned w = t01 | (t23 << 16);
          if (s2 > 0) w ^= 0x80808080u;
          dig[s2][q4] = w;
          q[s2] = __builtin_amdgcn_sdot4((int)w, (int)w, q[s2], false);
        }
        q[STAT_D0D1] = __builtin_amdgcn_sdot4((int)dig[0][q4], (int)dig[1][q4], q[STAT_D0D1], false);
      }
#pragma unroll
      for (int s2 = 0; s2 < NP; s2++) {
        any[s2] |= dig[s2][0] | dig[s2][1] | dig[s2][2] | dig[s2][3];
        if (s2 < ALWAYS_WRITTEN_PLANES) {
          signed char* piece = planes + ((s2 * groups + G) * (int64_t)nk + kt) * 1024;
          *(i32x4*)(piece + h * 512 + r * 16) = (i32x4){(int)dig[s2][0], (int)dig[s2][1], (int)dig[s2][2], (int)dig[s2][3]};
        } else {
#pragma unroll
          for (int i = 0; i < 4; i++) deep_dig[h][s2 - ALWAYS_WRITTEN_PLANES][i] = dig[s2][i];
        }
      }
    }
    const unsigned present = write_piece_mask(any, zmask, (int64_t)kt * groups + G);
#pragma unroll
    for (int s2 = ALWAYS_WRITTEN_PLANES; s2 < NP; s2++)
      if ((present >> s2) != 0) {
        signed char* piece = planes + ((s2 * groups + G) * (int64_t)nk + kt) * 1024;
#pragma unroll
        for (int h = 0; h < 2; h++)
          *(i32x4*)(piece + h * 512 + r * 16) = (i32x4){(int)deep_dig[h][s2 - ALWAYS_WRITTEN_PLANES][0], (int)deep_dig[h][s2 - ALWAYS_WRITTEN_PLANES][1],
                                                        (int)deep_dig[h][s2 - ALWAYS_WRITTEN_PLANES][2], (int)deep_dig[h][s2 - ALWAYS_WRITTEN_PLANES][3]};
      }
  }
  __syncthreads();
#pragma unroll
  for (int i = 0; i <= NSTAT; i++)
    if (q[i]) atomicAdd(&st_lds[i][f], q[i]);
  __syncthreads();
  if (threadIdx.x < 128) {
    unsigned long long* o = stats + f0 + threadIdx.x;
#pragma unroll
    for (int i = 0; i < STAT_COUNTS; i++) {
      const int val = st_lds[i][threadIdx.x];
      if (val) atomicAdd(o + (int64_t)i * n, (unsigned long long)(long long)val);
    }
    const unsigned long long counts = (unsigned long long)(unsigned)st_lds[NSTAT - 1][threadIdx.x] |
                                      ((unsigned long long)(unsigned)st_lds[NSTAT][threadIdx.x] << 32);
    if (counts) atomicAdd(o + (int64_t)STAT_COUNTS * n, counts);
  }
}

}

int enqueue_split(const I8Call& c, int i) {
  const I8Stat& s = c.stat[i];
  const int n = s.n, nk = c.nk;
  MDG_HIP(hipMemsetAsync(s.emax, 0, ints_bytes(n), c.st));
  if (s.vec()) {
    const int64_t slabs = std::min(ceil_div(c.n_tokens, (int64_t)64), std::max((int64_t)1, (int64_t)MDG_COLMAX_WGS / (n / 128)));
    const int64_t rows_vec = ceil_div(ceil_div(c.n_tokens, slabs), (int64_t)16) * 16;
    MDG_I8_DISPATCH(c, i8_colmax_vec_kernel, dim3((unsigned)(n / 128), (unsigned)ceil_div(c.n_tokens, rows_vec)), dim3(256), 0, c.st, s.x,
                       s.ld, c.n_tokens, rows_vec, s.emax);
    MDG_I8_DISPATCH(c, i8_split_vec_kernel, dim3((unsigned)(n / 128), (unsigned)ceil_div(nk, 2 * SPLIT_TILES)), dim3(256), 0, c.st, s.x,
                       s.ld, c.n_tokens, n, nk, s.emax, s.planes, s.stats(), s.zmask);
  } else {
    const int64_t rows_per_block = 2048;
    MDG_I8_DISPATCH(c, i8_colmax_kernel, dim3((unsigned)ceil_div(n, 64), (unsigned)ceil_div(c.n_tokens, rows_per_block)), dim3(256), 0,
                       c.st, s.x, s.ld, c.n_tokens, n, rows_per_block, s.emax);
    MDG_I8_DISPATCH(c, i8_split_kernel, dim3((unsigned)(n / 32), (unsigned)ceil_div(nk, SPLIT_STEPS)), dim3(256), 0, c.st, s.x, s.ld,
                       c.n_tokens, n, nk, s.emax, s.planes, s.stats(), s.zmask);
  }
  MDG_LAUNCH_CHECK();
  return MDG_OK;
}

}
```

Baseline: 1.188.

## Batch split, route, column and fallback covariance kernels across problems into single launches

Replaces the per-problem loops of split, colmax, route, column and fallback covariance launches with multi-problem kernels that index a flat work list covering every problem. Per-problem emax/stat buffers are laid out contiguously so a single memset clears them. The colmax kernel now uses packed u16 max over raw bits, and the split kernel prefetches the next tile while the current one is processed. Together these cut launch count and small-grid underutilisation, at the cost of per-block problem lookup and more complex workspace layout.

```diff
diff --git a/modegpt_amd/csrc/common.hpp b/modegpt_amd/csrc/common.hpp
--- a/modegpt_amd/csrc/common.hpp
+++ b/modegpt_amd/csrc/common.hpp
@@ -29,6 +29,9 @@
 int cov_accum_gated(const void* x, int dtype, int64_t n_tokens, int64_t n_feat, int64_t batch, int64_t ld, int relu, double* sigma,
                     int64_t ld_sigma, int64_t sigma_bs, void* ws, size_t ws_bytes, const int* gate, int gate_mask, int gate_want,
                     void* stream);
+size_t cov_accum_gated_multi_ws_bytes(int count, const mdg_cov_problem* pr);
+int cov_accum_gated_multi(int count, const mdg_cov_problem* pr, int dtype, int relu, void* ws, size_t ws_bytes, const int* gates,
+                          int gate_mask, int gate_want, void* stream);
 #define MDG_CHECK_ARG(cond, ...)            \
   do {                                      \
     if (!(cond)) {                          \
diff --git a/modegpt_amd/csrc/cov.hip b/modegpt_amd/csrc/cov.hip
--- a/modegpt_amd/csrc/cov.hip
+++ b/modegpt_amd/csrc/cov.hip
@@ -273,6 +273,44 @@
   double* sg = a.sigma + (int64_t)b * a.sigma_bs;
   const int64_t tile_stride = (int64_t)gridDim.x * (TILE * TILE);
   const double* pt = a.partial + (int64_t)blockIdx.x * (TILE * TILE);
+  const int e = blockIdx.y * 256 + threadIdx.x;
+  const int r = e / TILE, c = e % TILE;
+  const int64_t gr = (int64_t)bi * TILE + r, gc = (int64_t)bj * TILE + c;
+  if (gr >= a.n_feat || gc >= a.n_feat) return;
+  double s = 0.;
+  for (int k = 0; k < a.ksplit; k++) s += pt[k * tile_stride + e];
+  sg[gr * a.ld_sigma + gc] += s;
+}
+
+template <int DT, bool RELU, bool FAST>
+__global__ __launch_bounds__(256, 2) void cov_accum_gated_multi_kernel(CovMulti m) {
+  __shared__ double lds[4 * PANEL];
+  int u = blockIdx.x, pi = 0;
+  while (pi + 1 < m.n && u >= m.unit_start[pi + 1]) pi++;
+  u -= m.unit_start[pi];
+  const CovArgs& a = m.p[pi];
+  if ((int)blockIdx.y >= a.ksplit) return;
+  if (a.gate && (*a.gate & a.gate_mask) != a.gate_want) return;
+  const int b = u / a.ntri, t = u % a.ntri;
+  int bi, bj;
+  tri_decode(t, bi, bj);
+  if (bi == bj) cov_tile<DT, RELU, FAST, true>(a, lds, b, bi, bj, blockIdx.y, u);
+  else cov_tile<DT, RELU, FAST, false>(a, lds, b, bi, bj, blockIdx.y, u);
+}
+
+__global__ __launch_bounds__(256) void cov_reduce_multi_kernel(CovMulti m) {
+  int u = blockIdx.x, pi = 0;
+  while (pi + 1 < m.n && u >= m.unit_start[pi + 1]) pi++;
+  u -= m.unit_start[pi];
+  const CovArgs& a = m.p[pi];
+  if (a.ksplit <= 1) return;
+  if (a.gate && (*a.gate & a.gate_mask) != a.gate_want) return;
+  const int b = u / a.ntri, t = u % a.ntri;
+  int bi, bj;
+  tri_decode(t, bi, bj);
+  double* sg = a.sigma + (int64_t)b * a.sigma_bs;
+  const int64_t tile_stride = (int64_t)a.batch * a.ntri * (TILE * TILE);
+  const double* pt = a.partial + (int64_t)u * (TILE * TILE);
   const int e = blockIdx.y * 256 + threadIdx.x;
   const int r = e / TILE, c = e % TILE;
   const int64_t gr = (int64_t)bi * TILE + r, gc = (int64_t)bj * TILE + c;
@@ -413,10 +451,9 @@
                               stream);
 }
 
-int mdg::cov_accum_gated(const void* x, int dtype, int64_t n_tokens, int64_t n_feat, int64_t batch, int64_t ld, int relu,
-                         double* sigma, int64_t ld_sigma, int64_t sigma_bs, void* ws, size_t ws_bytes, const int* gate,
-                         int gate_mask, int gate_want, void* stream) {
-  MDG_CLEAR();
+static int cov_plan(const void* x, int dtype, int64_t n_tokens, int64_t n_feat, int64_t batch, int64_t ld, double* sigma,
+                    int64_t ld_sigma, int64_t sigma_bs, void* ws, size_t ws_bytes, const int* gate, int gate_mask, int gate_want,
+                    CovArgs& a, bool* fast) {
   MDG_CHECK_ARG(n_tokens >= 0 && n_feat > 0 && batch > 0, "mdg_cov_accum: bad sizes (tokens=%lld feat=%lld batch=%lld)",
                 (long long)n_tokens, (long long)n_feat, (long long)batch);
   MDG_CHECK_ARG(dtype >= MDG_BF16 && dtype <= MDG_F64, "mdg_cov_accum: unknown dtype %d", dtype);
@@ -426,10 +463,9 @@
   MDG_CHECK_ARG(batch == 1 || sigma_bs >= n_feat * ld_sigma - (ld_sigma - n_feat),
                 "mdg_cov_accum: sigma batch stride too small");
   MDG_CHECK_ARG(n_feat < (1 << 30) && batch * n_feat < (1ll << 31), "mdg_cov_accum: n_feat too large");
+  *fast = false;
   if (n_tokens == 0) return MDG_OK;
   MDG_CHECK_ARG(x && sigma, "mdg_cov_accum: null pointer");
-  hipStream_t st = (hipStream_t)stream;
-  CovArgs a;
   a.x = x;
   a.ld = ld;
   a.n_tokens = n_tokens;
@@ -452,7 +488,19 @@
     MDG_CHECK_ARG(ws && ws_bytes >= need, "mdg_cov_accum: workspace %zu < required %zu", ws_bytes, need);
   }
   MDG_CHECK_ARG((int64_t)a.batch * a.ntri < (1ll << 31) && a.ksplit < 65536, "mdg_cov_accum: grid too large");
-  const bool fast = a.vec_ok && (n_feat % TILE == 0);
+  *fast = a.vec_ok && (n_feat % TILE == 0);
+  return MDG_OK;
+}
+
+int mdg::cov_accum_gated(const void* x, int dtype, int64_t n_tokens, int64_t n_feat, int64_t batch, int64_t ld, int relu,
+                         double* sigma, int64_t ld_sigma, int64_t sigma_bs, void* ws, size_t ws_bytes, const int* gate,
+                         int gate_mask, int gate_want, void* stream) {
+  MDG_CLEAR();
+  CovArgs a;
+  bool fast = false;
+  MDG_TRY(cov_plan(x, dtype, n_tokens, n_feat, batch, ld, sigma, ld_sigma, sigma_bs, ws, ws_bytes, gate, gate_mask, gate_want, a, &fast));
+  if (n_tokens == 0) return MDG_OK;
+  hipStream_t st = (hipStream_t)stream;
   switch (dtype) {
     case MDG_BF16: launch_cov<MDG_BF16>(a, relu, fast, st); break;
     case MDG_F16: launch_cov<MDG_F16>(a, relu, fast, st); break;
@@ -463,6 +511,69 @@
   if (a.ksplit > 1) {
     hipLaunchKernelGGL(cov_reduce_kernel, dim3(a.batch * a.ntri, TILE * TILE / 256), dim3(256), 0, st, a);
     MDG_LAUNCH_CHECK();
+  }
+  return MDG_OK;
+}
+
+template <int DT>
+static void launch_cov_gated_multi(const CovMulti& m, dim3 grid, int relu, bool fast, hipStream_t st) {
+  if (fast) {
+    if (relu) hipLaunchKernelGGL((cov_accum_gated_multi_kernel<DT, true, true>), grid, dim3(256), 0, st, m);
+    else hipLaunchKernelGGL((cov_accum_gated_multi_kernel<DT, false, true>), grid, dim3(256), 0, st, m);
+  } else {
+    if (relu) hipLaunchKernelGGL((cov_accum_gated_multi_kernel<DT, true, false>), grid, dim3(256), 0, st, m);
+    else hipLaunchKernelGGL((cov_accum_gated_multi_kernel<DT, false, false>), grid, dim3(256), 0, st, m);
+  }
+}
+
+size_t mdg::cov_accum_gated_multi_ws_bytes(int count, const mdg_cov_problem* pr) {
+  size_t need = 0;
+  for (int i = 0; i < count; i++) need += align_up(mdg_cov_accum_ws_bytes(pr[i].n_tokens, pr[i].n_feat, pr[i].batch), 256);
+  return need;
+}
+
+int mdg::cov_accum_gated_multi(int count, const mdg_cov_problem* pr, int dtype, int relu, void* ws, size_t ws_bytes, const int* gates,
+                               int gate_mask, int gate_want, void* stream) {
+  MDG_CLEAR();
+  MDG_CHECK_ARG(count >= 1 && count <= MULTI_MAX && pr, "cov_accum_gated_multi: 1..%d problems", MULTI_MAX);
+  MDG_CHECK_ARG(dtype == MDG_BF16 || dtype == MDG_F16, "cov_accum_gated_multi: bf16 or fp16");
+  MDG_CHECK_ARG(ws_bytes >= cov_accum_gated_multi_ws_bytes(count, pr), "cov_accum_gated_multi: workspace too small");
+  hipStream_t st = (hipStream_t)stream;
+  CovArgs args[MULTI_MAX];
+  bool fast[MULTI_MAX];
+  size_t off = 0;
+  for (int i = 0; i < count; i++) {
+    const mdg_cov_problem& q = pr[i];
+    const size_t bytes = align_up(mdg_cov_accum_ws_bytes(q.n_tokens, q.n_feat, q.batch), 256);
+    MDG_TRY(cov_plan(q.x, dtype, q.n_tokens, q.n_feat, q.batch, q.ld, q.sigma, q.ld_sigma, q.sigma_batch_stride, (char*)ws + off, bytes,
+                     gates + i, gate_mask, gate_want, args[i], &fast[i]));
+    off += bytes;
+  }
+  if (pr[0].n_tokens == 0) return MDG_OK;
+  for (int f = 1; f >= 0; f--) {
+    CovMulti m;
+    m.n = 0;
+    int64_t units = 0;
+    int max_split = 1;
+    for (int i = 0; i < count; i++) {
+      if ((int)fast[i] != f) continue;
+      m.unit_start[m.n] = (int)units;
+      m.p[m.n++] = args[i];
+      units += (int64_t)args[i].batch * args[i].ntri;
+      max_split = std::max(max_split, args[i].ksplit);
+    }
+    if (!m.n) continue;
+    MDG_CHECK_ARG(units < (1ll << 31), "cov_accum_gated_multi: grid too large");
+    for (int i = m.n; i <= MULTI_MAX; i++) m.unit_start[i] = (int)units;
+    for (int i = m.n; i < MULTI_MAX; i++) m.p[i] = m.p[0];
+    const dim3 grid((unsigned)units, (unsigned)max_split);
+    if (dtype == MDG_BF16) launch_cov_gated_multi<MDG_BF16>(m, grid, relu, f != 0, st);
+    else launch_cov_gated_multi<MDG_F16>(m, grid, relu, f != 0, st);
+    MDG_LAUNCH_CHECK();
+    if (max_split > 1) {
+      hipLaunchKernelGGL(cov_reduce_multi_kernel, dim3((unsigned)units, TILE * TILE / 256), dim3(256), 0, st, m);
+      MDG_LAUNCH_CHECK();
+    }
   }
   return MDG_OK;
 }
diff --git a/modegpt_amd/csrc/cov_i8.hip b/modegpt_amd/csrc/cov_i8.hip
--- a/modegpt_amd/csrc/cov_i8.hip
+++ b/modegpt_amd/csrc/cov_i8.hip
@@ -6,15 +6,22 @@
 namespace {
 
 size_t layout(int count, const mdg_cov_problem* pr, void* ws, I8Call* out, size_t* fallback_off) {
-  size_t off = SHARED_BYTES + PARTIAL_BYTES, fb = 0;
+  size_t off = SHARED_BYTES, fb = 0;
   char* const base = (char*)ws;
+  int* emax_of[MAX_PROBLEMS];
+  for (int i = 0; i < count; i++) {
+    emax_of[i] = (int*)(base ? base + off : nullptr);
+    off += align_up(ints_bytes(pr[i].n_feat * pr[i].batch), 256);
+  }
   if (out) {
     out->count = count;
     out->n_tokens = pr[0].n_tokens;
     out->nk = (int)ceil_div(pr[0].n_tokens, KS);
     out->shared = (SharedBlock*)base;
-    out->partial = (double*)(base + SHARED_BYTES);
+    out->zero_bytes = off;
+    out->partial = (double*)(base + off);
   }
+  off += PARTIAL_BYTES;
   for (int i = 0; i < count; i++) {
     const int64_t cols = pr[i].n_feat * pr[i].batch, T = pr[i].n_tokens;
     const LoWsBytes lo = lo_ws_bytes(T, cols);
@@ -25,7 +32,7 @@
     s.route_flag = out ? out->shared->route_flag + i : nullptr;
     auto take = [&](size_t bytes) { char* p = base ? base + off : nullptr; off += bytes; return p; };
     s.planes = (signed char*)take(align_up((size_t)NP * (size_t)cols * (size_t)ceil_div(T, KS) * KS, 256));
-    s.emax = (int*)take(align_up(ints_bytes(cols), 256));
+    s.emax = emax_of[i];
     s.vals = (double*)take(align_up(route_vals_bytes(cols), 256));
     s.route = (RouteOut*)take(align_up(sizeof(RouteOut), 256));
     s.colpart = (double*)take(align_up(column_partials_bytes(cols), 256));
@@ -36,8 +43,8 @@
     s.lo_rentries = (LoEntry*)take(lo.rentries);
     s.lo_rtotals = (int*)take(align_up(lo.rtotals, 256));
     if (out) out->stat[i] = s;
-    fb = std::max(fb, mdg_cov_accum_ws_bytes(T, pr[i].n_feat, pr[i].batch));
   }
+  fb = cov_accum_gated_multi_ws_bytes(count, pr);
   if (fallback_off) *fallback_off = off;
   return off + fb + 256;
 }
@@ -91,20 +98,14 @@
   c.st = (hipStream_t)stream;
   c.f16 = (flags & MDG_I8_F16) != 0;
   c.relu = (flags & MDG_I8_RELU) != 0;
-  MDG_HIP(hipMemsetAsync(c.shared, 0, SHARED_BYTES, c.st));
-  for (int i = 0; i < count; i++) {
-    MDG_TRY(enqueue_split(c, i));
-    MDG_TRY(enqueue_route(c, i, tolerance));
-  }
+  MDG_TRY(enqueue_split(c));
+  MDG_TRY(enqueue_route(c, tolerance));
   if (offer_exact) MDG_TRY(enqueue_lo_lists(c, exact_always));
   MDG_TRY(enqueue_products(c, offer_exact, ev_start, ev_stop));
   if (offer_exact) MDG_TRY(enqueue_lo_products(c, exact_always));
-  for (int i = 0; i < count; i++) MDG_TRY(enqueue_columns(c, i));
-  for (int i = 0; i < count; i++) {
-    const mdg_cov_problem& q = problems[i];
-    MDG_TRY(cov_accum_gated(q.x, c.f16 ? MDG_F16 : MDG_BF16, c.n_tokens, q.n_feat, q.batch, q.ld, c.relu ? 1 : 0, q.sigma, q.ld_sigma, q.sigma_batch_stride, (char*)ws + fb_off,
-                            ws_bytes - fb_off, c.stat[i].route_flag, 2, 2, stream));
-  }
+  MDG_TRY(enqueue_columns(c));
+  MDG_TRY(cov_accum_gated_multi(count, problems, c.f16 ? MDG_F16 : MDG_BF16, c.relu ? 1 : 0, (char*)ws + fb_off, ws_bytes - fb_off,
+                                c.shared->route_flag, 2, 2, stream));
   MDG_TRY(report_product_diagnostics(c));
   if (used_i8) {
     int pf[MAX_PROBLEMS] = {};
diff --git a/modegpt_amd/csrc/cov_i8.hpp b/modegpt_amd/csrc/cov_i8.hpp
--- a/modegpt_amd/csrc/cov_i8.hpp
+++ b/modegpt_amd/csrc/cov_i8.hpp
@@ -135,6 +135,7 @@
   I8Stat stat[MAX_PROBLEMS];
   bool f16, relu;
   SharedBlock* shared;
+  size_t zero_bytes;
   double* partial;
   int* route_counts;
   hipStream_t st;
@@ -143,11 +144,11 @@
 inline size_t ints_bytes(int64_t n) { return (size_t)((n + 1) / 2 * 2) * sizeof(int) + (size_t)(NSTAT * n) * sizeof(unsigned long long) + sizeof(RouteScratch); }
 
 #pragma GCC visibility push(hidden)
-int enqueue_split(const I8Call& c, int i);
+int enqueue_split(const I8Call& c);
 size_t route_vals_bytes(int64_t n);
 size_t column_partials_bytes(int64_t n);
-int enqueue_route(const I8Call& c, int i, double tolerance);
-int enqueue_columns(const I8Call& c, int i);
+int enqueue_route(const I8Call& c, double tolerance);
+int enqueue_columns(const I8Call& c);
 struct LoWsBytes { size_t entries, counts, xd, rentries, rtotals; };
 LoWsBytes lo_ws_bytes(int64_t n_tokens, int64_t n);
 int enqueue_lo_lists(const I8Call& c, bool always);
diff --git a/modegpt_amd/csrc/cov_i8_route.hip b/modegpt_amd/csrc/cov_i8_route.hip
--- a/modegpt_amd/csrc/cov_i8_route.hip
+++ b/modegpt_amd/csrc/cov_i8_route.hip
@@ -47,9 +47,9 @@
   unsigned min_nnz;
 };
 
-__global__ __launch_bounds__(ROUTE_THREADS) void i8_route_kernel(const unsigned long long* __restrict__ stats, int* emax, int n, int64_t n_tokens,
-                                                                 double* __restrict__ vals, RoutePartial* partial, RouteScratch* scratch,
-                                                                 int* flag, RouteOut* out, int* route_counts, double tolerance) {
+__device__ __forceinline__ void route_statistic(const unsigned long long* __restrict__ stats, int* emax, int n, int64_t n_tokens,
+                                                double* __restrict__ vals, RoutePartial* partial, RouteScratch* scratch, int* flag,
+                                                RouteOut* out, int* route_counts, double tolerance, const unsigned nwg) {
   __shared__ unsigned long long group_max[NVAL][64];
   __shared__ Top2 wave_top[ROUTE_THREADS / 64][NVAL];
   __shared__ Top2 top[NVAL];
@@ -127,9 +127,8 @@
   __syncthreads();
   if (tid == 0) my_ticket = atomicAdd(&scratch->ticket, 1);
   __syncthreads();
-  if (my_ticket != (int)gridDim.x - 1) return;
+  if (my_ticket != (int)nwg - 1) return;
   __threadfence();
-  const unsigned nwg = gridDim.x;
   if (tid < NVAL) {
     Top2 r = partial[0].top[tid];
     unsigned w = 1;
@@ -288,8 +287,40 @@
   for (int j = tid; j < n; j += ROUTE_THREADS) emax[j] &= 255;
 }
 
-__global__ __launch_bounds__(256) void i8_clear_columns_kernel(const RouteOut* route, const int* flag, const int* emax, signed char* planes,
-                                                               unsigned char* zmask, int n, int nk) {
+struct RouteStat {
+  const unsigned long long* stats;
+  int* emax;
+  double* vals;
+  RoutePartial* partial;
+  RouteScratch* scratch;
+  int* flag;
+  RouteOut* out;
+  int n;
+  signed char* planes;
+  unsigned char* zmask;
+};
+struct RouteArgs {
+  RouteStat s[MAX_PROBLEMS];
+  int64_t n_tokens;
+  int* route_counts;
+  double tolerance;
+  int nk;
+};
+__global__ __launch_bounds__(ROUTE_THREADS) void i8_route_kernel(RouteArgs a) {
+  const RouteStat& s = a.s[blockIdx.y];
+  const unsigned nwg = (unsigned)((s.n + ROUTE_THREADS - 1) / ROUTE_THREADS);
+  if (blockIdx.x >= nwg) return;
+  route_statistic(s.stats, s.emax, s.n, a.n_tokens, s.vals, s.partial, s.scratch, s.flag, s.out, a.route_counts, a.tolerance, nwg);
+}
+
+__global__ __launch_bounds__(256) void i8_clear_columns_kernel(RouteArgs a) {
+  const RouteStat& s = a.s[blockIdx.z];
+  const RouteOut* route = s.out;
+  const int* flag = s.flag;
+  const int* emax = s.emax;
+  signed char* planes = s.planes;
+  unsigned char* zmask = s.zmask;
+  const int n = s.n, nk = a.nk;
   if ((*flag & 2) || (int)blockIdx.x >= route->n_out) return;
   const int j = route->out[blockIdx.x];
   const int64_t groups = n / 32;
@@ -321,11 +352,21 @@
   const RouteOut* route;
   const int* flag;
   double* part;
+  const int* emax;
+  double* sigma;
+  int64_t ld_sigma;
+  int block;
 };
+struct ColCall {
+  ColArgs s[MAX_PROBLEMS];
+};
 
 template <class EL, bool RELU>
-__global__ __launch_bounds__(64) void i8_columns_kernel(ColArgs a) {
-  const int pass = blockIdx.z;
+__global__ __launch_bounds__(64) void i8_columns_kernel(ColCall call) {
+  constexpr int PASSES = ROUTE_JMAX / COLK_GROUP;
+  const ColArgs& a = call.s[blockIdx.z / PASSES];
+  const int pass = blockIdx.z % PASSES;
+  if ((int)blockIdx.x * COLK_WG_COLS >= a.n) return;
   const int n_out = a.route->n_out;
   if ((*a.flag & 2) || pass * COLK_GROUP >= n_out) return;
   const int nj = min(COLK_GROUP, n_out - pass * COLK_GROUP);
@@ -399,7 +440,12 @@
     }
 }
 
-__global__ __launch_bounds__(256) void i8_columns_reduce_kernel(ColArgs a, const int* emax, double* sigma, int64_t ld_sigma, int block) {
+__global__ __launch_bounds__(256) void i8_columns_reduce_kernel(ColCall call) {
+  const ColArgs& a = call.s[blockIdx.z];
+  const int* emax = a.emax;
+  double* sigma = a.sigma;
+  const int64_t ld_sigma = a.ld_sigma;
+  const int block = a.block;
   const int k = blockIdx.y;
   if ((*a.flag & 2) || k >= a.route->n_out) return;
   const int c = blockIdx.x * 256 + threadIdx.x;
@@ -418,30 +464,48 @@
 size_t route_vals_bytes(int64_t n) { return (size_t)(NVAL * n) * sizeof(double) + (size_t)ceil_div(n, (int64_t)ROUTE_THREADS) * sizeof(RoutePartial); }
 size_t column_partials_bytes(int64_t n) { return (size_t)ROUTE_JMAX * COLK_CHUNKS * (size_t)n * sizeof(double); }
 
-int enqueue_route(const I8Call& c, int i, double tolerance) {
-  const I8Stat& s = c.stat[i];
-  const int n = s.n;
-  RoutePartial* partial = (RoutePartial*)(s.vals + (size_t)NVAL * n);
-  RouteScratch* scratch = (RouteScratch*)(s.stats() + (size_t)NSTAT * n);
-  hipLaunchKernelGGL(i8_route_kernel, dim3((unsigned)ceil_div(n, ROUTE_THREADS)), dim3(ROUTE_THREADS), 0, c.st, s.stats(), s.emax, n,
-                     c.n_tokens, s.vals, partial, scratch, s.route_flag, s.route, c.route_counts, tolerance);
-  hipLaunchKernelGGL(i8_clear_columns_kernel, dim3(ROUTE_JMAX, (unsigned)std::min(64, (c.nk + 3) / 4)), dim3(256), 0, c.st,
-                     (const RouteOut*)s.route, (const int*)s.route_flag, (const int*)s.emax, s.planes, s.zmask, n, c.nk);
+int enqueue_route(const I8Call& c, double tolerance) {
+  RouteArgs a;
+  a.n_tokens = c.n_tokens;
+  a.route_counts = c.route_counts;
+  a.tolerance = tolerance;
+  a.nk = c.nk;
+  int max_n = 0;
+  for (int i = 0; i < c.count; i++) {
+    const I8Stat& s = c.stat[i];
+    RouteStat& r = a.s[i];
+    r.stats = s.stats(); r.emax = s.emax; r.vals = s.vals; r.n = s.n;
+    r.partial = (RoutePartial*)(s.vals + (size_t)NVAL * s.n);
+    r.scratch = (RouteScratch*)(s.stats() + (size_t)NSTAT * s.n);
+    r.flag = s.route_flag; r.out = s.route;
+    r.planes = s.planes; r.zmask = s.zmask;
+    max_n = std::max(max_n, s.n);
+  }
+  for (int i = c.count; i < MAX_PROBLEMS; i++) a.s[i] = a.s[0];
+  hipLaunchKernelGGL(i8_route_kernel, dim3((unsigned)ceil_div(max_n, ROUTE_THREADS), (unsigned)c.count), dim3(ROUTE_THREADS), 0, c.st, a);
+  hipLaunchKernelGGL(i8_clear_columns_kernel, dim3(ROUTE_JMAX, (unsigned)std::min(64, (c.nk + 3) / 4), (unsigned)c.count), dim3(256), 0, c.st, a);
   MDG_LAUNCH_CHECK();
   return MDG_OK;
 }
 
-int enqueue_columns(const I8Call& c, int i) {
-  const I8Stat& s = c.stat[i];
-  ColArgs a;
-  a.x = s.x; a.ld = s.ld; a.T = c.n_tokens; a.n = s.n;
-  a.vec = s.vec();
-  a.route = s.route;
-  a.flag = s.route_flag;
-  a.part = s.colpart;
-  MDG_I8_DISPATCH(c, i8_columns_kernel, dim3((unsigned)ceil_div(s.n, COLK_WG_COLS), COLK_CHUNKS, ROUTE_JMAX / COLK_GROUP), dim3(64), 0, c.st, a);
-  hipLaunchKernelGGL(i8_columns_reduce_kernel, dim3((unsigned)ceil_div(s.n, 256), ROUTE_JMAX), dim3(256), 0, c.st, a, (const int*)s.emax, s.sigma,
-                     s.ld_sigma, s.block);
+int enqueue_columns(const I8Call& c) {
+  ColCall call;
+  int max_n = 0;
+  for (int i = 0; i < c.count; i++) {
+    const I8Stat& s = c.stat[i];
+    ColArgs& a = call.s[i];
+    a.x = s.x; a.ld = s.ld; a.T = c.n_tokens; a.n = s.n;
+    a.vec = s.vec();
+    a.route = s.route;
+    a.flag = s.route_flag;
+    a.part = s.colpart;
+    a.emax = s.emax; a.sigma = s.sigma; a.ld_sigma = s.ld_sigma; a.block = s.block;
+    max_n = std::max(max_n, s.n);
+  }
+  for (int i = c.count; i < MAX_PROBLEMS; i++) call.s[i] = call.s[0];
+  MDG_I8_DISPATCH(c, i8_columns_kernel, dim3((unsigned)ceil_div(max_n, COLK_WG_COLS), COLK_CHUNKS, (unsigned)(c.count * (ROUTE_JMAX / COLK_GROUP))),
+                     dim3(64), 0, c.st, call);
+  hipLaunchKernelGGL(i8_columns_reduce_kernel, dim3((unsigned)ceil_div(max_n, 256), ROUTE_JMAX, (unsigned)c.count), dim3(256), 0, c.st, call);
   MDG_LAUNCH_CHECK();
   return MDG_OK;
 }
diff --git a/modegpt_amd/csrc/cov_i8_split.hip b/modegpt_amd/csrc/cov_i8_split.hip
--- a/modegpt_amd/csrc/cov_i8_split.hip
+++ b/modegpt_amd/csrc/cov_i8_split.hip
@@ -4,6 +4,32 @@
 
 namespace mdg {
 namespace {
+
+struct SplitStat {
+  const bf16_t* x;
+  int64_t ld;
+  int* emax;
+  signed char* planes;
+  unsigned long long* stats;
+  unsigned char* zmask;
+  int n, cblocks;
+  int wg0_max, wg0_split;
+};
+struct SplitArgs {
+  SplitStat s[MAX_PROBLEMS];
+  int count, nk;
+  int64_t T, rows;
+  int steps;
+};
+__device__ __forceinline__ const SplitStat& split_work(const SplitArgs& a, bool split_pass, int& cb, int& slab) {
+  int p = 0;
+  while (p + 1 < a.count && (int)blockIdx.x >= (split_pass ? a.s[p + 1].wg0_split : a.s[p + 1].wg0_max)) p++;
+  const SplitStat& s = a.s[p];
+  const int local = (int)blockIdx.x - (split_pass ? s.wg0_split : s.wg0_max);
+  cb = local % s.cblocks;
+  slab = local / s.cblocks;
+  return s;
+}
 
 template <class EL>
 __device__ __forceinline__ long long fixed_point(int sig, int sh, bool& rounded) {
@@ -15,11 +41,16 @@
 }
 
 template <class EL, bool RELU>
-__global__ __launch_bounds__(256) void i8_colmax_kernel(const bf16_t* x, int64_t ld, int64_t T, int n, int64_t rows_per_block,
-                                                        int* emax) {
-  const int j = blockIdx.x * 64 + (threadIdx.x & 63);
-  const int64_t t0 = (int64_t)blockIdx.y * rows_per_block + (threadIdx.x >> 6);
-  const int64_t t1 = min(T, (int64_t)(blockIdx.y + 1) * rows_per_block);
+__global__ __launch_bounds__(256) void i8_colmax_kernel(SplitArgs a) {
+  int cb, slab;
+  const SplitStat& s = split_work(a, false, cb, slab);
+  const bf16_t* x = s.x;
+  const int64_t ld = s.ld, T = a.T;
+  const int n = s.n;
+  int* emax = s.emax;
+  const int j = cb * 64 + (threadIdx.x & 63);
+  const int64_t t0 = (int64_t)slab * a.rows + (threadIdx.x >> 6);
+  const int64_t t1 = min(T, (int64_t)(slab + 1) * a.rows);
   int best = 1;
   if (j < n)
     for (int64_t t = t0; t < t1; t += 4) {
@@ -44,11 +75,18 @@
 
 constexpr int SPLIT_STEPS = 64;
 template <class EL, bool RELU>
-__global__ __launch_bounds__(256) void i8_split_kernel(const bf16_t* x, int64_t ld, int64_t T, int n, int nk, const int* emax,
-                                                       signed char* planes, unsigned long long* stats, unsigned char* zmask) {
+__global__ __launch_bounds__(256) void i8_split_kernel(SplitArgs a) {
   __shared__ unsigned long long st_lds[NSTAT][32];
+  int G, slab;
+  const SplitStat& ss = split_work(a, true, G, slab);
+  const bf16_t* x = ss.x;
+  const int64_t ld = ss.ld, T = a.T;
+  const int n = ss.n, nk = a.nk;
+  const int* emax = ss.emax;
+  signed char* planes = ss.planes;
+  unsigned long long* stats = ss.stats;
+  unsigned char* zmask = ss.zmask;
   const int r = threadIdx.x & 31;
-  const int G = blockIdx.x;
   const int j = G * 32 + r;
   const int E = emax[j];
   const int64_t groups = n / 32;
@@ -56,7 +94,7 @@
   __syncthreads();
   long long q[NSTAT] = {};
   for (int kq = 0; kq < SPLIT_STEPS; kq += 8) {
-    const int kt = blockIdx.y * SPLIT_STEPS + kq + (threadIdx.x >> 5);
+    const int kt = slab * SPLIT_STEPS + kq + (threadIdx.x >> 5);
     if (kt >= nk) break;
     unsigned any[NP] = {};
 #pragma unroll
@@ -103,38 +141,57 @@
 #ifndef MDG_COLMAX_WGS
 #define MDG_COLMAX_WGS 4096
 #endif
+typedef unsigned short u16x2 __attribute__((ext_vector_type(2)));
+__device__ __forceinline__ unsigned pk_max_u16(unsigned a, unsigned b) {
+  return __builtin_bit_cast(unsigned, __builtin_elementwise_max(__builtin_bit_cast(u16x2, a), __builtin_bit_cast(u16x2, b)));
+}
 template <class EL, bool RELU>
-__global__ __launch_bounds__(256) void i8_colmax_vec_kernel(const bf16_t* x, int64_t ld, int64_t T, int64_t rows_per_block, int* emax) {
-  __shared__ int best_lds[128];
+__global__ __launch_bounds__(256) void i8_colmax_vec_kernel(SplitArgs a) {
+  __shared__ unsigned best_lds[128];
+  int cb, slab;
+  const SplitStat& s = split_work(a, false, cb, slab);
   const int cg = threadIdx.x & 15, tl = threadIdx.x >> 4;
-  const int j0 = blockIdx.x * 128 + cg * 8;
-  const int64_t t0 = (int64_t)blockIdx.y * rows_per_block + tl;
-  const int64_t t1 = min(T, (int64_t)(blockIdx.y + 1) * rows_per_block);
-  if (threadIdx.x < 128) best_lds[threadIdx.x] = 1;
-  __syncthreads();
-  int best[8] = {1, 1, 1, 1, 1, 1, 1, 1};
-  for (int64_t t = t0; t < t1; t += 16) {
-    const i32x4 v = *(const i32x4*)(x + t * ld + j0);
-#pragma unroll
-    for (int q = 0; q < 4; q++) {
-      const unsigned w = relu_pair<EL, RELU>((unsigned)v[q]);
-      best[2 * q] = max(best[2 * q], EL::ee_if_nonzero(w & 0xFFFF));
-      best[2 * q + 1] = max(best[2 * q + 1], EL::ee_if_nonzero(w >> 16));
-    }
-  }
-#pragma unroll
-  for (int q = 0; q < 8; q++) atomicMax(&best_lds[cg * 8 + q], best[q]);
-  __syncthreads();
-  if (threadIdx.x < 128) atomicMax(emax + blockIdx.x * 128 + threadIdx.x, best_lds[threadIdx.x]);
+  const bf16_t* xc = s.x + cb * 128 + cg * 8;
+  const int64_t ld = s.ld;
+  const int64_t t1 = min(a.T, (int64_t)(slab + 1) * a.rows);
+  int64_t t = (int64_t)slab * a.rows + tl;
+  if (threadIdx.x < 128) best_lds[threadIdx.x] = 0u;
+  __syncthreads();
+  unsigned best[4] = {0u, 0u, 0u, 0u};
+  auto take = [&](const i32x4& v) {
+#pragma unroll
+    for (int q = 0; q < 4; q++) best[q] = pk_max_u16(best[q], relu_pair<EL, RELU>((unsigned)v[q]) & 0x7FFF7FFFu);
+  };
+  for (; t + 48 < t1; t += 64) {
+    const i32x4 v0 = *(const i32x4*)(xc + t * ld), v1 = *(const i32x4*)(xc + (t + 16) * ld), v2 = *(const i32x4*)(xc + (t + 32) * ld),
+                v3 = *(const i32x4*)(xc + (t + 48) * ld);
+    take(v0); take(v1); take(v2); take(v3);
+  }
+  for (; t < t1; t += 16) take(*(const i32x4*)(xc + t * ld));
+#pragma unroll
+  for (int q = 0; q < 4; q++) {
+    atomicMax(&best_lds[cg * 8 + 2 * q], best[q] & 0xFFFFu);
+    atomicMax(&best_lds[cg * 8 + 2 * q + 1], best[q] >> 16);
+  }
+  __syncthreads();
+  if (threadIdx.x < 128) atomicMax(s.emax + cb * 128 + threadIdx.x, max(1, EL::ee_if_nonzero(best_lds[threadIdx.x])));
 }
 
 constexpr int SPLIT_TILES = 8;
 template <class EL, bool RELU>
-__global__ __launch_bounds__(256) void i8_split_vec_kernel(const bf16_t* x, int64_t ld, int64_t T, int n, int nk, const int* emax,
-                                                           signed char* planes, unsigned long long* stats, unsigned char* zmask) {
+__global__ __launch_bounds__(256) void i8_split_vec_kernel(SplitArgs a) {
   __shared__ __attribute__((aligned(16))) bf16_t tile[64 * 128];
   __shared__ int st_lds[NSTAT + 1][128];
-  const int f0 = blockIdx.x * 128;
+  int cb, slab;
+  const SplitStat& ss = split_work(a, true, cb, slab);
+  const bf16_t* x = ss.x;
+  const int64_t ld = ss.ld, T = a.T;
+  const int n = ss.n, nk = a.nk;
+  const int* emax = ss.emax;
+  signed char* planes = ss.planes;
+  unsigned long long* stats = ss.stats;
+  unsigned char* zmask = ss.zmask;
+  const int f0 = cb * 128;
   const int f = threadIdx.x & 127, ks = threadIdx.x >> 7;
   const int E = emax[f0 + f];
   const int64_t groups = n / 32;
@@ -151,16 +208,15 @@
       if (t < T) v[c4] = *(const i32x4*)(x + t * ld + f0 + (c & 15) * 8);
     }
   };
-  const int tile0 = blockIdx.y * SPLIT_TILES, tiles = (nk + 1) / 2;
-  for (int it = 0; it < SPLIT_TILES && tile0 + it < tiles; it++) {
+  const int tile0 = slab * a.steps, tiles = (nk + 1) / 2;
+  i32x4 v[4];
+  load_tile(tile0, v);
+  for (int it = 0; it < a.steps && tile0 + it < tiles; it++) {
     __syncthreads();
-    {
-      i32x4 v[4];
-      load_tile(tile0 + it, v);
-#pragma unroll
-      for (int c4 = 0; c4 < 4; c4++) *(i32x4*)(tile + (threadIdx.x + 256 * c4) * 8) = v[c4];
-    }
+#pragma unroll
+    for (int c4 = 0; c4 < 4; c4++) *(i32x4*)(tile + (threadIdx.x + 256 * c4) * 8) = v[c4];
     __syncthreads();
+    if (it + 1 < a.steps && tile0 + it + 1 < tiles) load_tile(tile0 + it + 1, v);
     const int kt = (tile0 + it) * 2 + ks;
     if (kt >= nk) continue;
     unsigned any[NP] = {};
@@ -240,23 +296,63 @@
 
 }
 
-int enqueue_split(const I8Call& c, int i) {
-  const I8Stat& s = c.stat[i];
-  const int n = s.n, nk = c.nk;
-  MDG_HIP(hipMemsetAsync(s.emax, 0, ints_bytes(n), c.st));
-  if (s.vec()) {
-    const int64_t slabs = std::min(ceil_div(c.n_tokens, (int64_t)64), std::max((int64_t)1, (int64_t)MDG_COLMAX_WGS / (n / 128)));
-    const int64_t rows_vec = ceil_div(ceil_div(c.n_tokens, slabs), (int64_t)16) * 16;
-    MDG_I8_DISPATCH(c, i8_colmax_vec_kernel, dim3((unsigned)(n / 128), (unsigned)ceil_div(c.n_tokens, rows_vec)), dim3(256), 0, c.st, s.x,
-                       s.ld, c.n_tokens, rows_vec, s.emax);
-    MDG_I8_DISPATCH(c, i8_split_vec_kernel, dim3((unsigned)(n / 128), (unsigned)ceil_div(nk, 2 * SPLIT_TILES)), dim3(256), 0, c.st, s.x,
-                       s.ld, c.n_tokens, n, nk, s.emax, s.planes, s.stats(), s.zmask);
-  } else {
-    const int64_t rows_per_block = 2048;
-    MDG_I8_DISPATCH(c, i8_colmax_kernel, dim3((unsigned)ceil_div(n, 64), (unsigned)ceil_div(c.n_tokens, rows_per_block)), dim3(256), 0,
-                       c.st, s.x, s.ld, c.n_tokens, n, rows_per_block, s.emax);
-    MDG_I8_DISPATCH(c, i8_split_kernel, dim3((unsigned)(n / 32), (unsigned)ceil_div(nk, SPLIT_STEPS)), dim3(256), 0, c.st, s.x, s.ld,
-                       c.n_tokens, n, nk, s.emax, s.planes, s.stats(), s.zmask);
+int enqueue_split(const I8Call& c) {
+  MDG_HIP(hipMemsetAsync(c.shared, 0, c.zero_bytes, c.st));
+  const int nk = c.nk;
+  for (int vec = 1; vec >= 0; vec--) {
+    SplitArgs a;
+    a.count = 0;
+    a.nk = nk;
+    a.T = c.n_tokens;
+    int64_t cblocks = 0;
+    for (int i = 0; i < c.count; i++) {
+      const I8Stat& s = c.stat[i];
+      if ((int)s.vec() != vec) continue;
+      SplitStat& q = a.s[a.count++];
+      q.x = s.x; q.ld = s.ld; q.emax = s.emax; q.planes = s.planes; q.stats = s.stats(); q.zmask = s.zmask;
+      q.n = s.n;
+      cblocks += vec ? s.n / 128 : s.n / 32;
+    }
+    if (!a.count) continue;
+    for (int i = a.count; i < MAX_PROBLEMS; i++) a.s[i] = a.s[0];
+    int64_t wg_max = 0, wg_split = 0;
+    if (vec) {
+      const int64_t slabs = std::min(ceil_div(c.n_tokens, (int64_t)64), std::max((int64_t)1, ceil_div((int64_t)MDG_COLMAX_WGS, cblocks)));
+      a.rows = ceil_div(ceil_div(c.n_tokens, slabs), (int64_t)16) * 16;
+      const int64_t tiles = ceil_div((int64_t)nk, (int64_t)2);
+      a.steps = SPLIT_TILES;
+      while (a.steps > 1 && cblocks * ceil_div(tiles, (int64_t)a.steps) < MDG_COLMAX_WGS) a.steps /= 2;
+      for (int i = 0; i < a.count; i++) {
+        SplitStat& q = a.s[i];
+        q.cblocks = q.n / 128;
+        q.wg0_max = (int)wg_max;
+        q.wg0_split = (int)wg_split;
+        wg_max += q.cblocks * ceil_div(c.n_tokens, a.rows);
+        wg_split += q.cblocks * ceil_div(tiles, (int64_t)a.steps);
+      }
+      MDG_CHECK_ARG(wg_max < (1ll << 31) && wg_split < (1ll << 31), "mdg_cov_accum_i8_multi: work list too long");
+      MDG_I8_DISPATCH(c, i8_colmax_vec_kernel, dim3((unsigned)wg_max), dim3(256), 0, c.st, a);
+      MDG_I8_DISPATCH(c, i8_split_vec_kernel, dim3((unsigned)wg_split), dim3(256), 0, c.st, a);
+    } else {
+      a.rows = 2048;
+      a.steps = SPLIT_STEPS;
+      for (int i = 0; i < a.count; i++) {
+        SplitStat& q = a.s[i];
+        q.cblocks = (int)ceil_div(q.n, 64);
+        q.wg0_max = (int)wg_max;
+        wg_max += q.cblocks * ceil_div(c.n_tokens, a.rows);
+      }
+      MDG_CHECK_ARG(wg_max < (1ll << 31), "mdg_cov_accum_i8_multi: work list too long");
+      MDG_I8_DISPATCH(c, i8_colmax_kernel, dim3((unsigned)wg_max), dim3(256), 0, c.st, a);
+      for (int i = 0; i < a.count; i++) {
+        SplitStat& q = a.s[i];
+        q.cblocks = q.n / 32;
+        q.wg0_split = (int)wg_split;
+        wg_split += q.cblocks * ceil_div((int64_t)nk, (int64_t)SPLIT_STEPS);
+      }
+      MDG_CHECK_ARG(wg_split < (1ll << 31), "mdg_cov_accum_i8_multi: work list too long");
+      MDG_I8_DISPATCH(c, i8_split_kernel, dim3((unsigned)wg_split), dim3(256), 0, c.st, a);
+    }
   }
   MDG_LAUNCH_CHECK();
   return MDG_OK;
```

Measured after the change: 1.199 (median of 6 runs). No clear change (+0.9%).
